# ferdean/lsa-fw

Hardware: AMD Instinct MI355X
Metric: converged eigenpairs/sec (k=20, shift-invert) (higher is better)
Workload: dtype c128

## Files before the change

### include/lsa_hip.h

```cpp
#ifndef LSA_HIP_H
#define LSA_HIP_H

#include <stdint.h>

#ifdef __cplusplus
extern "C" {
#endif

typedef enum { LSA_F64 = 0, LSA_C128 = 1 } lsa_dtype;

typedef enum {
    LSA_OK = 0,
    LSA_ERR_ARG = -1,
    LSA_ERR_HIP = -2,
    LSA_ERR_ZERO_PIVOT = -3,
    LSA_ERR_DIVERGED = -4,
    LSA_ERR_NONFINITE = -5,
    LSA_ERR_TIMEOUT = -6,
    LSA_ERR_COMM = -7,
    LSA_ERR_OOM = -8
} lsa_status;

typedef struct lsa_ctx lsa_ctx;
typedef struct lsa_mat lsa_mat;
// ... 11 lines not shown
    double max_rel_res;
    double seconds_factor;
    double seconds_solve;
    int32_t stagnated_solves;
    int32_t pc_fallback;
    int32_t backward_accepted;
    int32_t analysis_reused;
    int32_t refined_solves;
    int32_t reserved0;
} lsa_stats;

int lsa_ctx_create(int device, lsa_ctx **out);
void lsa_ctx_destroy(lsa_ctx *ctx);
const char *lsa_last_error(const lsa_ctx *ctx);
int lsa_ctx_synchronize(lsa_ctx *ctx);
int lsa_ctx_mem_info(lsa_ctx *ctx, int64_t *free_bytes, int64_t *total_bytes);
const char *lsa_ctx_arch(const lsa_ctx *ctx);

int lsa_vec_create(lsa_ctx *ctx, int64_t n, int dtype, lsa_vec **out);
void lsa_vec_destroy(lsa_vec *v);
int lsa_vec_upload(lsa_ctx *ctx, lsa_vec *v, const void *host);
int lsa_vec_download(lsa_ctx *ctx, const lsa_vec *v, void *host);

int lsa_csr_upload(lsa_ctx *ctx, int32_t n, int64_t nnz, const int32_t *rowptr, const int32_t *col,
                   const void *val, int dtype, lsa_mat **out);
void lsa_mat_destroy(lsa_mat *m);
int lsa_mat_download_values(lsa_ctx *ctx, const lsa_mat *m, void *host_val);
int lsa_csr_axpby(lsa_ctx *ctx, const lsa_mat *A, const lsa_mat *B, const double alpha[2], const double beta[2],
                  int out_dtype, lsa_mat **out);
int lsa_csr_window(lsa_ctx *ctx, const lsa_mat *M, const double *left, const double *right, lsa_mat **out);
int lsa_spmv(lsa_ctx *ctx, const lsa_mat *A, const lsa_vec *x, lsa_vec *y);
int lsa_spmv_transpose(lsa_ctx *ctx, const lsa_mat *A, int conj, const lsa_vec *x, lsa_vec *y);
int lsa_spmv_info(lsa_ctx *ctx, const lsa_mat *A, int xdtype, char *kernel, int32_t kernel_len, int64_t *bytes_moved);
int lsa_spmv_time(lsa_ctx *ctx, const lsa_mat *A, const lsa_vec *x, lsa_vec *y, int iters, double *avg_ms);

int lsa_ilu_create(lsa_ctx *ctx, const lsa_mat *C, int levels, double shift_tol, lsa_ilu **out);
void lsa_ilu_destroy(lsa_ilu *pc);
int lsa_ilu_set_algorithm(lsa_ctx *ctx, lsa_ilu *pc, int algo, int32_t block_size);
int lsa_ilu_solve(lsa_ctx *ctx, lsa_ilu *pc, int which, const lsa_vec *b, lsa_vec *x);
int lsa_ilu_solve_time(lsa_ctx *ctx, lsa_ilu *pc, int which, const lsa_vec *b, lsa_vec *x, int iters, double *avg_ms);
int lsa_ilu_info(const lsa_ilu *pc, int64_t *nnz, int32_t *levels_lower, int32_t *levels_upper, int32_t *nshift);
int lsa_ilu_download(lsa_ctx *ctx, const lsa_ilu *pc, int32_t *rowptr, int32_t *col, void *val);

typedef struct lsa_nd_sym lsa_nd_sym;
typedef struct lsa_ndlu lsa_ndlu;
int lsa_nd_analyse(int32_t n, const int32_t *rowptr, const int32_t *col, int32_t leaf_size, const int8_t *constraint, lsa_nd_sym **out);
int lsa_nd_order(int32_t n, const int32_t *rowptr, const int32_t *col, int32_t leaf_size, const int8_t *constraint, lsa_nd_sym **out);
int lsa_nd_analyse_tree(int32_t n, const int32_t *rowptr, const int32_t *col, int32_t ntree, const int32_t *first, const int32_t *size,
                        const int32_t *parent, const int32_t *owner, int32_t rank, int32_t nranks, lsa_nd_sym **out);
const char *lsa_nd_sym_error(const lsa_nd_sym *h);
void lsa_nd_sym_destroy(lsa_nd_sym *h);
int lsa_nd_sym_info(const lsa_nd_sym *h, int32_t *ntree, int32_t *nlevels, int32_t *max_front, int64_t *index_entries,
                    int64_t *factor_entries, int64_t *front_entries, double *flops);
int lsa_nd_sym_memory(const lsa_nd_sym *h, int32_t scalar_bytes, int64_t work_budget_bytes, int64_t *out, int64_t *upd_off, int64_t *work_off,
                      int32_t *chunk_of);
int lsa_nd_sym_export(const lsa_nd_sym *h, int32_t *perm, int32_t *node_start, int32_t *parent, int32_t *level, int32_t *front_size,
                      int32_t *idx);
int lsa_nd_sym_export_tables(const lsa_nd_sym *h, int32_t *cmap, int32_t *gptr, int32_t *gidx, int64_t *asm_dst, int32_t *lvl_ptr,
                             int32_t *lvl_nodes);
int lsa_nd_sym_export_dist(const lsa_nd_sym *h, int32_t *kind, int64_t *front_off, int64_t *u_off, int32_t *asm_src, int32_t *children_ptr,
                           int32_t *children_idx, int64_t *scalars);
int lsa_nd_sym_export_top(const lsa_nd_sym *h, int32_t *owner, int32_t *rows, int64_t *exch, int64_t *totals);
int lsa_ndlu_create(lsa_ctx *ctx, const lsa_mat *C, int32_t leaf_size, lsa_ndlu **out);
int lsa_ndlu_prepare(lsa_ctx *ctx, const lsa_mat *P, int dtype, int32_t leaf_size, const int8_t *constraint);
int lsa_ndlu_prepare_tree(lsa_ctx *ctx, const lsa_mat *P, int dtype, int32_t ntree, const int32_t *first, const int32_t *size,
                          const int32_t *parent);
int lsa_ndlu_create_tree(lsa_ctx *ctx, const lsa_mat *C, int32_t ntree, const int32_t *first, const int32_t *size, const int32_t *parent,
                         const int32_t *owner, lsa_ndlu **out);
int lsa_ndlu_refactor(lsa_ctx *ctx, lsa_ndlu *f, const lsa_mat *C);
void lsa_ndlu_destroy(lsa_ndlu *f);
int lsa_ndlu_solve(lsa_ctx *ctx, lsa_ndlu *f, const lsa_vec *b, lsa_vec *x);
int lsa_ndlu_solve_batch(lsa_ctx *ctx, int32_t J, lsa_ndlu *const *f, const lsa_vec *const *b, lsa_vec *const *x);
int lsa_ndlu_solve_adjoint(lsa_ctx *ctx, lsa_ndlu *f, int conj, const lsa_vec *b, lsa_vec *x);
int lsa_ndlu_solve_time(lsa_ctx *ctx, lsa_ndlu *f, const lsa_vec *b, lsa_vec *x, int iters, double *avg_ms);
int lsa_ndlu_solve_multi(lsa_ctx *ctx, lsa_ndlu *f, int trans, int32_t nrhs, const lsa_vec *B, int64_t ldb, lsa_vec *X, int64_t ldx);
int lsa_ndlu_solve_multi_time(lsa_ctx *ctx, lsa_ndlu *f, int trans, int32_t nrhs, const lsa_vec *B, int64_t ldb, lsa_vec *X, int64_t ldx,
                              int iters, double *avg_ms);
int lsa_ndlu_set_multi_transposed(lsa_ctx *ctx, lsa_ndlu *f, int on);
int lsa_ndlu_multi_info(const lsa_ndlu *f, int32_t *width, int64_t *extra_bytes, int32_t *launches_per_pass);
int lsa_ndlu_inertia(lsa_ctx *ctx, lsa_ndlu *f, int64_t *negative, int64_t *zero, int64_t *positive);
int lsa_ndlu_prepared_memory(lsa_ctx *ctx, int64_t *out);
int lsa_ndlu_info(const lsa_ndlu *f, int32_t *ntree, int32_t *nlevels, int32_t *max_front, int64_t *factor_entries,
                  int64_t *front_entries, int64_t *apply_bytes, int32_t *apply_launches, double *seconds_analyse,
                  double *seconds_numeric);
int lsa_ndlu_sweep_level(const lsa_ndlu *f, int32_t level, int32_t *nodes, int32_t *max_pivot, int32_t *fwd_rows, int32_t *bwd_rows,
                         int32_t *fwd_tiles, int32_t *bwd_tiles);

int lsa_gmres(lsa_ctx *ctx, const lsa_mat *C, lsa_ilu *pc, const lsa_vec *b, lsa_vec *x, int use_x0, double rtol,
              int restart, int maxit, int32_t *iters, double *rel_res);

typedef struct {
    int32_t ilu_levels;
    double ilu_shift;
    double ksp_rtol;
    int32_t ksp_restart;
    int32_t ksp_maxit;
    int32_t pc_type;
    double antishift[2];
} lsa_op_options;

int lsa_op_create(lsa_ctx *ctx, const lsa_mat *A, const lsa_mat *M, const double sigma[2], int mode,
                  const lsa_op_options *opts, lsa_op **out);
void lsa_op_destroy(lsa_op *op);
int lsa_op_apply(lsa_ctx *ctx, lsa_op *op, const lsa_vec *x, lsa_vec *y);
int lsa_op_stats(const lsa_op *op, lsa_stats *out);
int lsa_op_set_adjoint(lsa_ctx *ctx, lsa_op *op, int on);
int lsa_op_set_projection(lsa_ctx *ctx, lsa_op *op, const double *keep);

int lsa_krylov_create(lsa_ctx *ctx, lsa_op *op, int32_t ncv, lsa_krylov **out);
void lsa_krylov_destroy(lsa_krylov *k);
int lsa_krylov_set_row_permutation(lsa_ctx *ctx, lsa_krylov *k, const int32_t *perm);
int lsa_krylov_set_start(lsa_ctx *ctx, lsa_krylov *k, const void *host_v);
int lsa_krylov_inject(lsa_ctx *ctx, lsa_krylov *k, int32_t j, const void *host_v);
int lsa_krylov_extend(lsa_ctx *ctx, lsa_krylov *k, int32_t j0, int32_t j1, void *H, int32_t ldh, int32_t *breakdown);
int lsa_krylov_restart(lsa_ctx *ctx, lsa_krylov *k, int32_t m, int32_t knew, const void *Q, int32_t ldq);
int lsa_krylov_ritz_vectors(lsa_ctx *ctx, lsa_krylov *k, int32_t m, int32_t nvec, const void *Y, int32_t ldy,
                            int normalise, void *X);
int lsa_krylov_imag_norms(const lsa_krylov *k, int32_t nvec, double *out);
int lsa_eig_residuals(lsa_ctx *ctx, const lsa_mat *A, const lsa_mat *M, int32_t nvec, const void *lam, const void *X,
                      double *res);
int lsa_eig_biorth(lsa_ctx *ctx, const lsa_mat *M, int64_t n, int32_t nvec, const void *X, const void *Z, void *G,
                   double *norm_z, double *norm_mx);

typedef enum {
    LSA_WHICH_LARGEST_MAGNITUDE = 1,
    LSA_WHICH_LARGEST_REAL = 3,
    LSA_WHICH_SMALLEST_REAL = 4,
    LSA_WHICH_LARGEST_IMAGINARY = 5,
    LSA_WHICH_SMALLEST_IMAGINARY = 6,
    LSA_WHICH_TARGET_MAGNITUDE = 7,
    LSA_WHICH_TARGET_REAL = 8,
    LSA_WHICH_TARGET_IMAGINARY = 9
} lsa_which;
typedef struct {
    int32_t nev;
    int32_t max_restarts;
    double tol;
    int32_t which;
    int32_t transform;
    double sigma[2];
    double antishift[2];
    double target[2];
    uint64_t seed;
    double keep_fraction;
} lsa_ks_options;
typedef struct {
    int32_t nconv;
    int32_t nout;
    int32_t restarts;
    int32_t pad;
    int64_t op_applies;
    double next_unconverged;
    double seconds_expand;
    double seconds_dense;
    double seconds_restart;
} lsa_ks_result;
int lsa_krylov_shape(const lsa_krylov *k, int64_t *n, int32_t *ncv);
int64_t lsa_mat_rows(const lsa_mat *m);
int lsa_krylov_solve(lsa_ctx *ctx, lsa_krylov *k, const lsa_ks_options *opts, const void *v0, const double *mask, int32_t max_out,
                     void *theta_out, void *lambda_out, void *X_out, double *est_out, lsa_ks_result *result);
typedef struct {
    int64_t rounds;
    int64_t launches;
    int64_t periods;
    double launches_per_round;
    int64_t lockstep_steps[16];
    int64_t solo_steps[16];
// ... 137 lines not shown
```

### lsa-fw_amd/csrc/ndlu.hip

```cpp
#include "ndlu_internal.h"

namespace {

void nd_free(lsa_ndlu* f) {
    if (!f) return;
    ndlu_multi_free(f);
    for (void* p : {f->d_top, (void*)f->d_top_icmap, (void*)f->d_top_jobs, (void*)f->d_top_tiles})
        if (p) (void)hipFree(p);
    for (void* p : {(void*)f->d_lnodes_bwd, (void*)f->d_dist_nodes, (void*)f->d_child_ptr, (void*)f->d_child_idx, f->d_xstage, f->d_xg, (void*)f->d_tgoff, f->d_tg})
        if (p) (void)hipFree(p);
    for (void* p : {(void*)f->d_nodes, (void*)f->d_lnodes, (void*)f->d_gell, (void*)f->d_idx, (void*)f->d_cmap, (void*)f->d_tiles,
                    (void*)f->d_chunk_nodes, (void*)f->d_asm_dst, (void*)f->d_asm_src, (void*)f->d_ipiv, (void*)f->d_rowq, (void*)f->d_flag, (void*)f->d_xflag, (void*)f->d_maxabs,
                    f->d_lfac, f->d_ufac, f->d_work, f->d_upd, f->d_ubuf, f->d_xb, f->d_acc, f->d_tmp, f->d_ybuf, (void*)f->d_cand[0], (void*)f->d_cand[1], f->d_dinv})
        if (p) (void)hipFree(p);
    if (f->ev_panel) (void)hipEventDestroy(f->ev_panel);
    if (f->ev_pivots) (void)hipEventDestroy(f->ev_pivots);
    if (f->side) (void)hipStreamDestroy(f->side);
    delete f;
}

int nd_setup_top(lsa_ctx* ctx, lsa_ndlu* f, const std::vector<NdNodeDev>& nodes) {
    const NdSymbolic& S = f->S;
    f->top = NdTop{};
    f->top_level = -1;
// ... 14 lines not shown
        const int32_t c = S.child_idx[(size_t)c0 + ci];
        const NdNodeDev& nd = nodes[(size_t)c];
        bool on_level = false;
        for (int32_t q = S.lvl_ptr[(size_t)lr - 1]; q < S.lvl_ptr[(size_t)lr]; ++q) on_level |= S.lvl_nodes[(size_t)q] == c;
        if (!on_level || nd.nchild < 1 || nd.acc_off < 0 || nd.f <= nd.m || nd.m < 1 || S.kind[(size_t)c] == 3 || S.kind[(size_t)c] == 4) return LSA_OK;
        tp.node[ci] = NdTopNode{nd.acc_off, nd.ge_off, nd.own0, nd.m, nd.f, nd.nchild, (int32_t)s, 0};
        s += nd.m;
        replaced += (int64_t)nd.m * nd.m + 2 * (int64_t)nd.m * (nd.f - nd.m);
    }
    const NdNodeDev& nr = nodes[(size_t)R];
    tp.node[K] = NdTopNode{nr.acc_off, nr.ge_off, nr.own0, mR, mR, K, (int32_t)s, 0};
    s += mR;
    if (s > limit) return LSA_OK;
    tp.s = (int32_t)s;
    std::vector<int32_t> icmap((size_t)K * mR, -1);
    for (int32_t ci = 0; ci < K; ++ci) {
        const int32_t c = S.child_idx[(size_t)c0 + ci];
        for (int32_t p = 0; p < S.f[(size_t)c] - S.m[(size_t)c]; ++p) {
            const int32_t k = S.cmap[(size_t)S.cmap_off[(size_t)c] + p];
            if (k < 0 || k >= mR) return LSA_OK;
            icmap[(size_t)ci * mR + k] = p;
        }
    }
    std::vector<NdTopJob> jobs;
    std::vector<int32_t> tiles;
    auto add = [&](const NdTopJob& jb) {
        for (int32_t ti = 0; ti < (jb.M + 31) / 32; ++ti)
            for (int32_t tj = 0; tj < (jb.N + 31) / 32; ++tj) {
                tiles.push_back((int32_t)jobs.size());
                tiles.push_back((ti << 16) | tj);
            }
        jobs.push_back(jb);
    };
    const int64_t oR = tp.node[K].off;
    add(NdTopJob{0, 0, oR * s + oR, nr.lfac_off, mR, mR, 0, 1, 1, mR, 0, 0, 0, 0});
    for (int32_t ci = 0; ci < K; ++ci) {
        const NdNodeDev& nd = nodes[(size_t)S.child_idx[(size_t)c0 + ci]];
        const int32_t m = nd.m, b = nd.f - nd.m;
        const int64_t o = tp.node[ci].off;
        add(NdTopJob{nd.ufac_off, nr.lfac_off, o * s + oR, -1, m, mR, b, b, mR, 0, 1, 2, nd.cmap_off, 1});
        add(NdTopJob{nr.lfac_off, nd.lfac_off + (int64_t)m * m, oR * s + o, -1, mR, m, b, mR, m, 0, 0, 1, nd.cmap_off, 0});
    }
    f->top_tiles[0] = (int32_t)tiles.size() / 2;
    for (int32_t ci = 0; ci < K; ++ci)
        for (int32_t di = 0; di < K; ++di) {
            const NdNodeDev &nc = nodes[(size_t)S.child_idx[(size_t)c0 + ci]], &nd = nodes[(size_t)S.child_idx[(size_t)c0 + di]];
            add(NdTopJob{tp.node[ci].off * s + oR, nd.lfac_off + (int64_t)nd.m * nd.m, tp.node[ci].off * s + tp.node[di].off, ci == di ? nc.lfac_off : -1, nc.m,
                         nd.m, nd.f - nd.m, (int32_t)s, nd.m, nc.m, 2, 1, nd.cmap_off, 0});
        }
    f->top_tiles[1] = (int32_t)tiles.size() / 2 - f->top_tiles[0];
    LSA_CHECK(upload(ctx, icmap, &f->d_top_icmap));
    LSA_CHECK(upload(ctx, jobs, &f->d_top_jobs));
    LSA_CHECK(upload(ctx, tiles, &f->d_top_tiles));
    LSA_HIP_ALLOC(ctx, hipMalloc(&f->d_top, (size_t)(s * s) * esize(f->dtype)));
    f->top = tp;
    f->top_level = lr;
    f->top_replaced_entries = replaced;
    f->solve_launches -= 2;
    return LSA_OK;
}


struct TileBuffer {
    std::vector<int32_t> tiles;
    void begin(TileList& tl) {
        tl.off = (int64_t)tiles.size() / 2;
        tl.count = 0;
    }
    void push(TileList& tl, int32_t a, int32_t b) {
        tiles.push_back(a);
        tiles.push_back(b);
        ++tl.count;
    }
};

void nd_setup_knobs(lsa_ndlu* f) {
    const char* e = getenv("LSA_ND_TP_MIN");
    f->tp_min = e && *e ? std::max(1, atoi(e)) : 512;
    const char* sbm = getenv("LSA_ND_SB_MIN");
    f->sb_min = std::max(f->tp_min, sbm && *sbm ? std::max(1, atoi(sbm)) : 1024);
    f->ycap = kNB;
    const char* sbc = getenv("LSA_ND_SB_COLS");
    f->sb_cols = sbc && *sbc ? std::min(1024, std::max(kGT, atoi(sbc) / kGT * kGT)) : kSB;
}

bool nd_setup_ordered(const NdSymbolic& S) {
    const bool dist = S.nranks > 1;
    bool ordered = true;
    for (size_t k = 0; k < S.perm.size() && ordered; ++k) ordered = S.perm[k] == (int32_t)k || dist;
    if (dist)
        for (int32_t t = 0; t < S.nt && ordered; ++t)
            for (int32_t r = 1; r < S.m[(size_t)t]; ++r)
                if (S.idx[(size_t)S.idx_off[(size_t)t] + r] != S.idx[(size_t)S.idx_off[(size_t)t]] + r) {
                    ordered = false;
                    break;
                }
    return ordered;
}

int64_t nd_setup_budget(const NdSymbolic& S, size_t es, int64_t free_agreed) {
    size_t free_b = 0, total_b = 0;
    if (hipMemGetInfo(&free_b, &total_b) != hipSuccess) free_b = (size_t)16 << 30;
    const int64_t after = (int64_t)free_b - S.factor_entries * (int64_t)es;
    int64_t budget = std::max<int64_t>(after / 4, (int64_t)256 << 20) / (int64_t)es;
    if (S.has_dist) budget = std::max<int64_t>((free_agreed > 0 ? free_agreed : (int64_t)free_b) / 6, (int64_t)256 << 20) / (int64_t)es;
    if (const char* e = getenv("LSA_ND_WORK_MB")) budget = std::max<int64_t>(atoll(e), 1) * (1 << 20) / (int64_t)es;
    return budget;
}

std::vector<NdNodeDev> nd_setup_nodes(const NdSymbolic& S, const NdMemoryPlan& P) {
    std::vector<NdNodeDev> nodes((size_t)S.nt);
    for (int32_t t = 0; t < S.nt; ++t) {
        NdNodeDev& nd = nodes[(size_t)t];
        nd.front_off = P.work_off[(size_t)t];
        nd.lfac_off = P.lfac_off[(size_t)t];
        nd.ufac_off = P.ufac_off[(size_t)t];
        nd.upd_off = P.upd_off[(size_t)t];
        nd.u_off = S.u_off[(size_t)t];
        nd.ge_off = S.ge_off[(size_t)t];
        nd.acc_off = P.acc_off[(size_t)t];
        nd.pacc_off = P.pacc_off[(size_t)t];
        nd.idx_off = (int32_t)S.idx_off[(size_t)t];
        nd.cmap_off = S.cmap_off[(size_t)t];
        nd.piv_off = S.piv_off[(size_t)t];
        nd.own0 = S.m[(size_t)t] > 0 ? S.idx[(size_t)S.idx_off[(size_t)t]] : 0;
        nd.m = S.m[(size_t)t];
        nd.f = S.f[(size_t)t];
        nd.parent = S.parent[(size_t)t];
        nd.nchild = S.child_ptr[(size_t)t + 1] - S.child_ptr[(size_t)t];
        nd.brow0 = S.brow0[(size_t)t];
        nd.brow = S.brow[(size_t)t];
        nd.orow0 = S.orow0[(size_t)t];
        nd.orows = S.orows[(size_t)t];
        nd.flags = S.kind[(size_t)t] == 4 ? 1 : 0;
        nd.pad0 = 0;
        nd.xg_base = S.xg_base[(size_t)t];
        nd.xg_stride = S.xg_stride[(size_t)t];
        nd.inv_off = S.kind[(size_t)t] == 4
                         ? nd.front_off + (int64_t)(S.m[(size_t)t] + nd_slice_width(S.f[(size_t)t] - S.m[(size_t)t], S.nranks)) * S.f[(size_t)t]
                         : -1;
    }
    return nodes;
}

std::vector<NdChunk> nd_setup_chunks(const NdSymbolic& S, const NdMemoryPlan& P, std::vector<int32_t>& chunk_of) {
    std::vector<NdChunk> chunks;
    chunk_of.assign((size_t)S.nt, -1);
    for (size_t c = 0; c + 1 < P.chunk_begin.size(); ++c) {
        NdChunk ch;
        ch.node_begin = P.chunk_begin[c];
        ch.node_count = P.chunk_begin[c + 1] - P.chunk_begin[c];
        ch.work_entries = P.chunk_work[c];
        ch.exchange_before = P.chunk_exchange_before[c] != 0;
        for (int32_t q = 0; q < ch.node_count; ++q) {
            const int32_t t = S.lvl_nodes[(size_t)ch.node_begin + q];
            ch.max_m = std::max(ch.max_m, S.m[(size_t)t]);
            ch.max_f = std::max(ch.max_f, S.f[(size_t)t]);
            ch.sorted_m.push_back(S.m[(size_t)t]);
            chunk_of[(size_t)t] = (int32_t)c;
        }
        chunks.push_back(std::move(ch));
    }
    return chunks;
}

int nd_setup_assembly(lsa_ctx* ctx, lsa_ndlu* f, const std::vector<NdNodeDev>& nodes, const std::vector<int32_t>& chunk_of) {
// ... 603 lines not shown
}

int lsa_ndlu_solve_multi(lsa_ctx* ctx, lsa_ndlu* f, int trans, int32_t nrhs, const lsa_vec* B, int64_t ldb, lsa_vec* X, int64_t ldx) {
    LSA_CHECK(nd_multi_check(ctx, "lsa_ndlu_solve_multi", f, trans, nrhs, B, ldb, X, ldx));
    LSA_CHECK(nd_multi_run(ctx, f, trans, nrhs, B, ldb, X, ldx));
    LSA_HIP_CHECK(ctx, hipStreamSynchronize(ctx->stream));
    return LSA_OK;
}

int lsa_ndlu_solve_multi_time(lsa_ctx* ctx, lsa_ndlu* f, int trans, int32_t nrhs, const lsa_vec* B, int64_t ldb, lsa_vec* X, int64_t ldx, int iters,
                              double* avg_ms) {
    if (!avg_ms || iters < 1) return lsa_set_error(ctx, LSA_ERR_ARG, "lsa_ndlu_solve_multi_time: bad argument");
    LSA_CHECK(nd_multi_check(ctx, "lsa_ndlu_solve_multi_time", f, trans, nrhs, B, ldb, X, ldx));
    if (B->d == X->d) return lsa_set_error(ctx, LSA_ERR_ARG, "lsa_ndlu_solve_multi_time: repeated solves need B and X apart");
    LSA_CHECK(nd_multi_run(ctx, f, trans, nrhs, B, ldb, X, ldx));
    LSA_HIP_CHECK(ctx, hipEventRecord(ctx->ev0, ctx->stream));
    for (int i = 0; i < iters; ++i) LSA_CHECK(nd_multi_run(ctx, f, trans, nrhs, B, ldb, X, ldx));
    LSA_HIP_CHECK(ctx, hipEventRecord(ctx->ev1, ctx->stream));
    LSA_HIP_CHECK(ctx, hipEventSynchronize(ctx->ev1));
    float ms = 0.f;
    LSA_HIP_CHECK(ctx, hipEventElapsedTime(&ms, ctx->ev0, ctx->ev1));
    *avg_ms = (double)ms / iters;
    return LSA_OK;
}

int lsa_ndlu_set_multi_transposed(lsa_ctx* ctx, lsa_ndlu* f, int on) {
    if (!ctx || !f) return lsa_set_error(ctx, LSA_ERR_ARG, "lsa_ndlu_set_multi_transposed: null argument");
    f->multi_transposed = on != 0;
    return LSA_OK;
}

int lsa_ndlu_multi_info(const lsa_ndlu* f, int32_t* width, int64_t* extra_bytes, int32_t* launches_per_pass) {
    if (!f) return LSA_ERR_ARG;
    if (width) *width = f->multi_width;
    if (extra_bytes) *extra_bytes = f->multi_bytes;
    if (launches_per_pass) *launches_per_pass = f->solve_launches;
    return LSA_OK;
}

int lsa_ndlu_inertia(lsa_ctx* ctx, lsa_ndlu* f, int64_t* negative, int64_t* zero, int64_t* positive) {
    if (!ctx || !f || !negative || !zero || !positive) return lsa_set_error(ctx, LSA_ERR_ARG, "lsa_ndlu_inertia: null argument");
    if (f->dtype != LSA_F64) return lsa_set_error(ctx, LSA_ERR_ARG, "lsa_ndlu_inertia: needs real factors (a real symmetric matrix)");
    if (f->S.nranks != 1) return lsa_set_error(ctx, LSA_ERR_ARG, "lsa_ndlu_inertia: not available for a forest cut over ranks");
    *negative = *zero = *positive = 0;
    const NdSymbolic& S = f->S;
    std::vector<double> blk;
    LSA_HIP_CHECK(ctx, hipStreamSynchronize(ctx->stream));
    for (int32_t t = 0; t < S.nt; ++t) {
        const int32_t m = S.m[(size_t)t];
        if (m <= 0) continue;
        blk.resize((size_t)m * m);
        LSA_HIP_CHECK(ctx, hipMemcpy(blk.data(), (const double*)f->d_lfac + f->h_lfac_off[(size_t)t], (size_t)m * m * sizeof(double), hipMemcpyDeviceToHost));
        int64_t ng = 0, ze = 0, ps = 0;
        const int rc = lsa_dense_sym_inertia(m, blk.data(), m, 1e-13, &ng, &ze, &ps);
        if (rc != LSA_OK) return lsa_set_error(ctx, rc, "lsa_ndlu_inertia: the pivot block of tree node %d holds non-finite values", t);
        *negative += ng;
        *zero += ze;
        *positive += ps;
    }
    return LSA_OK;
}

int lsa_ndlu_prepared_memory(lsa_ctx* ctx, int64_t* out) {
    if (!ctx || !out) return lsa_set_error(ctx, LSA_ERR_ARG, "lsa_ndlu_prepared_memory: null argument");
    const lsa_ndlu* c = ctx->nd_cache;
    if (!c) return lsa_set_error(ctx, LSA_ERR_ARG, "lsa_ndlu_prepared_memory: the context holds no prepared analysis");
    return nd_memory_report(c->S, (int32_t)esize(c->dtype), 0, out, nullptr, nullptr, nullptr);
}

int lsa_ndlu_sweep_level(const lsa_ndlu* f, int32_t level, int32_t* nodes, int32_t* max_pivot, int32_t* fwd_rows, int32_t* bwd_rows, int32_t* fwd_tiles,
                         int32_t* bwd_tiles) {
    if (!f || level < 0 || (size_t)level >= f->levels.size()) return LSA_ERR_ARG;
    const NdLevel& L = f->levels[(size_t)level];
    if (nodes) *nodes = L.node_count;
    if (max_pivot) *max_pivot = L.max_m;
    if (fwd_rows) *fwd_rows = L.sweep_rows;
    if (bwd_rows) *bwd_rows = L.bwd_rows;
    if (fwd_tiles) *fwd_tiles = L.fwd_tiles;
    if (bwd_tiles) *bwd_tiles = L.bwd_tiles;
    return LSA_OK;
}

int lsa_ndlu_info(const lsa_ndlu* f, int32_t* ntree, int32_t* nlevels, int32_t* max_front, int64_t* factor_entries, int64_t* front_entries,
                  int64_t* apply_bytes, int32_t* apply_launches, double* seconds_analyse, double* seconds_numeric) {
    if (!f) return LSA_ERR_ARG;
    const NdSymbolic& S = f->S;
    if (ntree) *ntree = S.nt;
    if (nlevels) *nlevels = S.nlevels;
    if (max_front) {
        int32_t mf = 0;
        for (int32_t v : S.f) mf = std::max(mf, v);
        *max_front = mf;
    }
    if (factor_entries) *factor_entries = S.factor_entries;
    if (front_entries) *front_entries = f->lfac_entries + f->ufac_entries + f->work_entries + f->upd_entries;
    const int64_t swept = S.factor_entries - f->top_replaced_entries * (f->top.s > 0) + (int64_t)f->top.s * f->top.s;
    if (apply_bytes) *apply_bytes = swept * (int64_t)esize(f->dtype) + 16 * (3 * (int64_t)S.n + 2 * S.u_off[(size_t)S.nt]);
    if (apply_launches) *apply_launches = f->solve_launches;
    if (seconds_analyse) *seconds_analyse = f->seconds_analyse;
    if (seconds_numeric) *seconds_numeric = f->seconds_numeric;
    return LSA_OK;
}

}
```

### lsa-fw_amd/csrc/ndlu_factor.hip

```cpp
#include "ndlu_internal.h"

namespace {

template <typename T>
__global__ __launch_bounds__(256) void nd_maxabs2_kernel(int64_t nnz, const T* __restrict__ v, unsigned long long* __restrict__ out) {
    __shared__ double wmax[4];
    double best = 0.0;
    const int64_t stride = (int64_t)gridDim.x * blockDim.x;
    for (int64_t i = (int64_t)blockIdx.x * blockDim.x + threadIdx.x; i < nnz; i += stride) {
        const double a = s_abs2(v[i]);
        if (a == a && a > best) best = a;
        else if (a != a) best = a;
    }
    for (int o = 32; o > 0; o >>= 1) {
        const double other = __shfl_xor(best, o);
        best = (best != best) ? best : (other != other) ? other : fmax(best, other);
    }
    if ((threadIdx.x & 63) == 0) wmax[threadIdx.x >> 6] = best;
    __syncthreads();
    if (threadIdx.x == 0) {
        for (int w = 1; w < 4; ++w) best = (best != best) ? best : (wmax[w] != wmax[w]) ? wmax[w] : fmax(best, wmax[w]);
        atomicMax(out, (unsigned long long)__double_as_longlong(best));
    }
}

template <typename T>
__global__ void nd_scale_kernel(int64_t count, T* __restrict__ v, double factor) {
    const int64_t stride = (int64_t)gridDim.x * blockDim.x;
    for (int64_t i = (int64_t)blockIdx.x * blockDim.x + threadIdx.x; i < count; i += stride) v[i] = s_mul(factor, v[i]);
}

template <typename T>
__global__ void nd_assemble_kernel(int64_t count, const T* __restrict__ val, const int32_t* __restrict__ src, const int64_t* __restrict__ dst,
                                   T* __restrict__ front) {
    const int64_t stride = (int64_t)gridDim.x * blockDim.x;
    for (int64_t e = (int64_t)blockIdx.x * blockDim.x + threadIdx.x; e < count; e += stride) front[dst[e]] = val[src[e]];
}

template <typename T>
__global__ __launch_bounds__(256) void nd_extend_add_kernel(const int32_t* __restrict__ tiles, const NdNodeDev* __restrict__ nodes,
                                                            const int32_t* __restrict__ cmap, T* __restrict__ front, const T* __restrict__ upd) {
    const int32_t c = tiles[2 * blockIdx.x], i0 = tiles[2 * blockIdx.x + 1];
    const NdNodeDev nc = nodes[c];
    const NdNodeDev np = nodes[nc.parent];
    const int32_t b = nc.f - nc.m;
    const int32_t* map = cmap + nc.cmap_off;
    const int32_t i = i0 + (threadIdx.x >> 4);
    if (i >= b) return;
    const T* src = upd + nc.upd_off + (int64_t)i * b;
    int32_t pr = map[i];
    if (pr >= np.m) {
        pr -= np.brow0;
        if (pr < np.m || pr >= np.m + np.brow) return;
    }
    T* dst = front + np.front_off + (int64_t)pr * np.f;
    for (int32_t j = threadIdx.x & 15; j < b; j += 16) {
        T* d = dst + map[j];
        *d = s_add(*d, src[j]);
    }
}

template <typename T>
__global__ __launch_bounds__(256) void nd_extend_add_staged_kernel(const NdNodeDev* __restrict__ nodes, const int32_t* __restrict__ cmap, T* __restrict__ front,
                                                                   const T* __restrict__ src, int32_t c, int32_t row0, int32_t nrows) {
    const NdNodeDev nc = nodes[c];
    const NdNodeDev np = nodes[nc.parent];
    const int32_t b = nc.f - nc.m;
    const int32_t* map = cmap + nc.cmap_off;
    const int32_t k = (int32_t)blockIdx.x * 16 + (threadIdx.x >> 4);
    if (k >= nrows) return;
    int32_t pr = map[row0 + k];
    if (pr >= np.m) {
        pr -= np.brow0;
        if (pr < np.m || pr >= np.m + np.brow) return;
    }
    const T* s = src + (int64_t)k * b;
    T* dst = front + np.front_off + (int64_t)pr * np.f;
    for (int32_t j = threadIdx.x & 15; j < b; j += 16) {
        T* d = dst + map[j];
        *d = s_add(*d, s[j]);
    }
}

template <int CTRL>
__device__ __forceinline__ unsigned long long dpp_mov_key(unsigned long long v) {
    const int lo = __builtin_amdgcn_update_dpp(0, (int)(unsigned)(v & 0xFFFFFFFFull), CTRL, 0xF, 0xF, false);
    const int hi = __builtin_amdgcn_update_dpp(0, (int)(unsigned)(v >> 32), CTRL, 0xF, 0xF, false);
    return ((unsigned long long)(unsigned)hi << 32) | (unsigned)lo;
}
__device__ __forceinline__ unsigned long long wave_max_key(unsigned long long v) {
    unsigned long long o;
    o = dpp_mov_key<0xB1>(v);
    v = o > v ? o : v;
    o = dpp_mov_key<0x4E>(v);
    v = o > v ? o : v;
    o = dpp_mov_key<0x141>(v);
    v = o > v ? o : v;
    o = dpp_mov_key<0x140>(v);
    v = o > v ? o : v;
    unsigned long long best = 0ull;
#pragma unroll
    for (int row = 0; row < 4; ++row) {
        const unsigned lo = (unsigned)__builtin_amdgcn_readlane((int)(unsigned)(v & 0xFFFFFFFFull), 16 * row);
        const unsigned hi = (unsigned)__builtin_amdgcn_readlane((int)(unsigned)(v >> 32), 16 * row);
        const unsigned long long r = ((unsigned long long)hi << 32) | lo;
        best = r > best ? r : best;
    }
    return best;
}

__device__ __forceinline__ unsigned long long pivot_key(double mag2, int32_t row) {
    return ((unsigned long long)__double_as_longlong(mag2) & ~0xFFFFull) | (unsigned long long)(65535 - row);
}


template <typename T, int NT, int RPT, int W>
__global__ __launch_bounds__(NT) void nd_gj_fused_kernel(const int32_t* __restrict__ lvl_nodes, const NdNodeDev* __restrict__ nodes,
                                                         T* __restrict__ front, int32_t* __restrict__ ipiv, int32_t* __restrict__ rowq,
                                                         int32_t kb, int32_t k0, int32_t kprev, int32_t* __restrict__ flag, double tiny2) {
    __shared__ unsigned long long skey[W];
    __shared__ T prow_s[2][W];
    __shared__ int32_t prows[W];
    __shared__ T yprev[W][16];
    __shared__ int32_t pprev[W];
    const int32_t t = lvl_nodes[blockIdx.x];
    const NdNodeDev nd = nodes[t];
    const int32_t m = nd.m, ld = nd.f;
    T* a = front + nd.front_off;
    const int tid = threadIdx.x, lane = tid & 63;
    const int32_t wp = kprev >= 0 ? min(W, m - kprev) : 0;
    if (blockIdx.y > 0) {
        if (wp <= 0) return;
        const int32_t cb = ((int32_t)blockIdx.y - 1) * 16 + (tid & 15);
        const int32_t c = kb + cb;
        const bool mine = cb < kNB && c < m && !(c >= kprev && c < kprev + wp) && !(k0 >= 0 && c >= k0 && c < k0 + W);
        if (tid < W) pprev[tid] = tid < wp ? ipiv[nd.piv_off + kprev + tid] : -1;
        __syncthreads();
        for (int e = tid; e < 16 * W; e += NT) {
            const int j = e >> 4;
            yprev[j][e & 15] = (mine && j < wp) ? a[(size_t)pprev[j] * ld + c] : scalar_traits<T>::zero();
        }
        __syncthreads();
        if (!mine) return;
        T y[W];
#pragma unroll
        for (int j = 0; j < W; ++j) y[j] = yprev[j][tid & 15];
        constexpr int RL = NT / 16;
        for (int32_t i0 = tid >> 4; i0 < m; i0 += 4 * RL) {
            T cur[4], mult[4][W];
#pragma unroll
            for (int u = 0; u < 4; ++u) {
                const int32_t i = i0 + u * RL;
                const T* ai = a + (size_t)min(i, m - 1) * ld;
                cur[u] = ai[c];
#pragma unroll
                for (int j = 0; j < W; ++j) mult[u][j] = j < wp ? ai[kprev + j] : scalar_traits<T>::zero();
            }
#pragma unroll
            for (int u = 0; u < 4; ++u) {
                const int32_t i = i0 + u * RL;
                if (i >= m) break;
                bool is_piv = false;
#pragma unroll
                for (int j = 0; j < W; ++j) is_piv |= (i == pprev[j]);
                T acc = is_piv ? scalar_traits<T>::zero() : cur[u];
#pragma unroll
                for (int j = 0; j < W; ++j) fma_acc(acc, mult[u][j], y[j]);
                a[(size_t)i * ld + c] = acc;
            }
        }
        return;
    }
    if (k0 < 0) return;
    const int32_t w = min(W, m - k0);
    if (w <= 0) return;
    int32_t* piv = ipiv + nd.piv_off;
    int32_t* rq = rowq + nd.piv_off;
    if (tid < W) {
        skey[tid] = 0ull;
        pprev[tid] = tid < wp ? piv[kprev + tid] : -1;
    }
    __syncthreads();
    if (wp > 0 && tid < W * W) {
        const int j = tid / W, cc = tid % W;
        yprev[j][cc] = (j < wp && cc < w) ? a[(size_t)pprev[j] * ld + k0 + cc] : scalar_traits<T>::zero();
    }
    T r[RPT][W];
    bool used[RPT];
#pragma unroll
    for (int q = 0; q < RPT; ++q) {
        const int32_t i = tid + NT * q;
        used[q] = i >= m || rq[min(i, m - 1)] >= 0;
#pragma unroll
        for (int c = 0; c < W; ++c) r[q][c] = (i < m && c < w) ? a[(size_t)i * ld + k0 + c] : scalar_traits<T>::zero();
    }
    __syncthreads();
    if (wp > 0) {
#pragma unroll
        for (int q = 0; q < RPT; ++q) {
            const int32_t i = tid + NT * q;
            if (i >= m) continue;
            bool is_piv = false;
#pragma unroll
            for (int j = 0; j < W; ++j) is_piv |= (i == pprev[j]);
            T mult[W];
#pragma unroll
            for (int j = 0; j < W; ++j) mult[j] = j < wp ? a[(size_t)i * ld + kprev + j] : scalar_traits<T>::zero();
#pragma unroll
            for (int c = 0; c < W; ++c) {
                T acc = is_piv ? scalar_traits<T>::zero() : r[q][c];
#pragma unroll
                for (int j = 0; j < W; ++j) fma_acc(acc, mult[j], yprev[j][c]);
                r[q][c] = c < w ? acc : scalar_traits<T>::zero();
            }
        }
    }
#pragma unroll
    for (int jj = 0; jj < W; ++jj) {
        if (jj >= w) break;
        unsigned long long key = 0ull;
#pragma unroll
        for (int q = 0; q < RPT; ++q) {
            if (!used[q]) {
                const unsigned long long kq = pivot_key(s_abs2(r[q][jj]), tid + NT * q);
                key = kq > key ? kq : key;
            }
        }
        key = wave_max_key(key);
        if (lane == 0) atomicMax(&skey[jj], key);
        __syncthreads();
        key = skey[jj];
        const int32_t p = 65535 - (int32_t)(key & 0xFFFFull);
        if (tid == 0) {
            piv[k0 + jj] = p;
            prows[jj] = p;
            if (!(__longlong_as_double((long long)(key & ~0xFFFFull)) > tiny2) && atomicCAS(&flag[1], 0, t + 1) == 0) {
                flag[2] = k0 + jj;
                flag[3] = (int32_t)(key >> 32);
            }
        }
#pragma unroll
        for (int q = 0; q < RPT; ++q) {
            if (tid + NT * q == p) {
                T pv = r[q][jj];
                if (s_abs2(pv) == 0.0) s_from(pv, 1.0, 0.0);
                const T pinv = s_inv(pv);
#pragma unroll
                for (int j = 0; j < W; ++j) {
                    const T v = (j == jj) ? pinv : s_mul(pinv, r[q][j]);
                    prow_s[jj & 1][j] = v;
                    r[q][j] = v;
                }
                used[q] = true;
                rq[p] = k0 + jj;
            }
        }
        __syncthreads();
        T prow[W];
#pragma unroll
        for (int j = 0; j < W; ++j) prow[j] = prow_s[jj & 1][j];
#pragma unroll
        for (int q = 0; q < RPT; ++q) {
            const int32_t i = tid + NT * q;
            if (i >= m || i == p) continue;
            const T fm = r[q][jj];
            if (s_abs2(fm) == 0.0) continue;
            const T nfm = s_sub(scalar_traits<T>::zero(), fm);
            r[q][jj] = scalar_traits<T>::zero();
#pragma unroll
            for (int j = 0; j < W; ++j) fma_acc(r[q][j], nfm, prow[j]);
        }
    }
#pragma unroll
    for (int q = 0; q < RPT; ++q) {
        const int32_t i = tid + NT * q;
        if (i < m) {
#pragma unroll
            for (int j = 0; j < W; ++j)
                if (j < w) a[(size_t)i * ld + k0 + j] = r[q][j];
        }
    }
}

template <typename T>
__global__ __launch_bounds__(256) void nd_gj_stage_kernel(const int32_t* __restrict__ lvl_nodes, const NdNodeDev* __restrict__ nodes,
                                                          const T* __restrict__ front, const int32_t* __restrict__ ipiv, int32_t kb, int32_t kw,
                                                          int32_t ycap, int32_t c_lo, int32_t c_hi, T* __restrict__ ybuf) {
    const int32_t t = lvl_nodes[blockIdx.x];
    const NdNodeDev nd = nodes[t];
    const int32_t m = nd.m, ld = nd.f;
    const int32_t nb = min(kw, m - kb);
    const int32_t c = c_lo + (int32_t)blockIdx.y * 256 + threadIdx.x;
    if (nb <= 0 || m <= kNB || c >= min(m, c_hi)) return;
    const T* a = front + nd.front_off;
    T* yb = ybuf + (size_t)ycap * nd.piv_off;
    const int32_t* pv = ipiv + nd.piv_off + kb;
    int32_t j = 0;
    for (; j + 4 <= nb; j += 4) {
        const T v0 = a[(size_t)pv[j] * ld + c], v1 = a[(size_t)pv[j + 1] * ld + c], v2 = a[(size_t)pv[j + 2] * ld + c], v3 = a[(size_t)pv[j + 3] * ld + c];
        yb[(size_t)j * m + c] = v0;
        yb[(size_t)(j + 1) * m + c] = v1;
        yb[(size_t)(j + 2) * m + c] = v2;
        yb[(size_t)(j + 3) * m + c] = v3;
    }
    for (; j < nb; ++j) yb[(size_t)j * m + c] = a[(size_t)pv[j] * ld + c];
}

template <typename T>
__global__ __launch_bounds__(256) void nd_gj_gemm_kernel(const int32_t* __restrict__ lvl_nodes, const NdNodeDev* __restrict__ nodes,
                                                         T* __restrict__ front, const int32_t* rowq, int32_t kb,
                                                         const T* __restrict__ ybuf, int32_t only_lo, int32_t only_hi, int32_t skip_lo,
                                                         int32_t skip_hi, int32_t ztile0) {
    __shared__ T Ws[kNB][kGT + 1];
    __shared__ T Ys[kNB][kGT + 1];
    const int32_t t = lvl_nodes[blockIdx.x];
    const NdNodeDev nd = nodes[t];
    const int32_t m = nd.m, ld = nd.f;
    const int32_t nb = min(kNB, m - kb);
    const int32_t row0 = (int32_t)blockIdx.y * kGT, col0 = ((int32_t)blockIdx.z + ztile0) * kGT;
    if (nb <= 0 || row0 >= m || col0 >= m) return;
    if (col0 >= kb && col0 + kGT <= kb + nb) return;
    if (only_hi > only_lo && (col0 >= only_hi || col0 + kGT <= only_lo)) return;
    if (col0 >= skip_lo && col0 + kGT <= skip_hi) return;
    T* a = front + nd.front_off;
    const T* yb = ybuf + (size_t)kNB * nd.piv_off;
    const int32_t* rq = rowq + nd.piv_off;
    const int tid = threadIdx.x, tx = tid & 15, ty = tid >> 4;
    for (int e = tid; e < kNB * kGT; e += 256) {
        const int qa = e / kNB, ja = e - qa * kNB;
        const int32_t gr = row0 + qa;
        Ws[ja][qa] = (ja < nb && gr < m) ? a[(size_t)gr * ld + kb + ja] : scalar_traits<T>::zero();
        const int jb = e / kGT, qb = e - jb * kGT;
        const int32_t gc = col0 + qb;
        Ys[jb][qb] = (jb < nb && gc < m) ? yb[(size_t)jb * m + gc] : scalar_traits<T>::zero();
    }
    __syncthreads();
    T acc[4][4];
#pragma unroll
    for (int i = 0; i < 4; ++i)
#pragma unroll
        for (int j = 0; j < 4; ++j) acc[i][j] = scalar_traits<T>::zero();
    for (int k = 0; k < nb; ++k) {
        T av[4], bv[4];
#pragma unroll
        for (int i = 0; i < 4; ++i) av[i] = Ws[k][ty * 4 + i];
#pragma unroll
        for (int j = 0; j < 4; ++j) bv[j] = Ys[k][tx + 16 * j];
#pragma unroll
        for (int i = 0; i < 4; ++i)
#pragma unroll
            for (int j = 0; j < 4; ++j) fma_acc(acc[i][j], av[i], bv[j]);
    }
#pragma unroll
    for (int i = 0; i < 4; ++i) {
        const int32_t gr = row0 + ty * 4 + i;
        if (gr >= m) continue;
        const int32_t q = rq[gr];
        const bool is_piv = q >= kb && q < kb + nb;
#pragma unroll
        for (int j = 0; j < 4; ++j) {
            const int32_t gc = col0 + tx + 16 * j;
            if (gc >= m || (gc >= kb && gc < kb + nb)) continue;
            if ((gc >= skip_lo && gc < skip_hi) || (only_hi > only_lo && (gc < only_lo || gc >= only_hi))) continue;
            T* cptr = a + (size_t)gr * ld + gc;
            *cptr = is_piv ? acc[i][j] : s_add(*cptr, acc[i][j]);
        }
    }
}

constexpr int kTA = 8;

template <typename T>
struct tp_first {
    static constexpr int RPT = sizeof(T) == 16 ? 1 : 2;
    static constexpr int rows = 256 * RPT;
};

__host__ __device__ inline int32_t tp_sets(int32_t m, int32_t first_rows, int32_t round) {
    int32_t n = (m + first_rows - 1) / first_rows;
    for (int32_t r = 0; r < round; ++r) n = (n + kTA - 1) / kTA;
    return n;
}

template <typename T, bool FIRST, bool LAST>
__global__ __launch_bounds__(256) void nd_tp_round_kernel(const int32_t* __restrict__ lvl_nodes, const NdNodeDev* __restrict__ nodes,
                                                          const T* __restrict__ front, int32_t* __restrict__ ipiv, int32_t* __restrict__ rowq, int32_t kb,
                                                          int32_t round, const int32_t* __restrict__ cand_in, int32_t* __restrict__ cand_out,
                                                          T* __restrict__ dinv, int32_t* __restrict__ flag, double tiny2) {
// ... 193 lines not shown
    }
    T* dst = front + nd.inv_off + (size_t)ra * m;
    const bool mine = ra >= nd.orow0 && ra < nd.orow0 + nd.orows;
    T* keep = lfac + nd.lfac_off + (size_t)(mine ? ra - nd.orow0 : 0) * m;
    for (int32_t cb = threadIdx.x & 15; cb < m; cb += 16) {
        const T v = src[q[cb]];
        dst[cb] = v;
        if (mine) keep[cb] = v;
    }
}

typedef double mfma_d4 __attribute__((ext_vector_type(4)));
__device__ __forceinline__ double plane_of(double v, int) { return v; }
__device__ __forceinline__ double plane_of(cplx v, int p) { return p == 0 ? v.re : v.im; }

template <typename T>
struct MfmaTile {
    static constexpr int BK = 16, LDAS = BK + 1, LDBS = kGT + 16, NPL = (int)(sizeof(T) / sizeof(double));
    double As[NPL][kGT * LDAS];
    double Bs[NPL][BK * LDBS];
};

template <typename T, typename FA, typename FB>
__device__ __forceinline__ void mfma_tile_product(int32_t K, FA loadA, FB loadB, MfmaTile<T>& sm, mfma_d4 (&acc)[MfmaTile<T>::NPL][2][2]) {
    constexpr int BK = MfmaTile<T>::BK, LDAS = MfmaTile<T>::LDAS, LDBS = MfmaTile<T>::LDBS, NPL = MfmaTile<T>::NPL;
    const int tid = threadIdx.x, lane = tid & 63, wave = tid >> 6;
    const int wr = 32 * (wave >> 1), wc = 32 * (wave & 1), l15 = lane & 15, l4 = lane >> 4;
#pragma unroll
    for (int p = 0; p < NPL; ++p)
#pragma unroll
        for (int i = 0; i < 2; ++i)
#pragma unroll
            for (int j = 0; j < 2; ++j) acc[p][i][j] = mfma_d4{0.0, 0.0, 0.0, 0.0};
    T pa[4], pb[4];
    auto gload = [&](int32_t kk) {
#pragma unroll
        for (int s = 0; s < 4; ++s) {
            const int e = tid + 256 * s;
            pa[s] = loadA(e >> 4, kk + (e & 15));
            pb[s] = loadB(kk + (e >> 6), e & 63);
        }
    };
    gload(0);
    for (int32_t kk = 0; kk < K; kk += BK) {
#pragma unroll
        for (int s = 0; s < 4; ++s) {
            const int e = tid + 256 * s;
#pragma unroll
            for (int p = 0; p < NPL; ++p) {
                sm.As[p][(e >> 4) * LDAS + (e & 15)] = plane_of(pa[s], p);
                sm.Bs[p][(e >> 6) * LDBS + (e & 63)] = plane_of(pb[s], p);
            }
        }
        __syncthreads();
        if (kk + BK < K) gload(kk + BK);
#pragma unroll
        for (int k4 = 0; k4 < BK; k4 += 4) {
            if (kk + k4 >= K) break;
            double a[NPL][2], bb[NPL][2];
#pragma unroll
            for (int p = 0; p < NPL; ++p)
#pragma unroll
                for (int i = 0; i < 2; ++i) {
                    a[p][i] = sm.As[p][(wr + 16 * i + l15) * LDAS + k4 + l4];
                    bb[p][i] = sm.Bs[p][(k4 + l4) * LDBS + wc + 16 * i + l15];
                }
#pragma unroll
            for (int i = 0; i < 2; ++i)
#pragma unroll
                for (int j = 0; j < 2; ++j) {
                    acc[0][i][j] = __builtin_amdgcn_mfma_f64_16x16x4f64(a[0][i], bb[0][j], acc[0][i][j], 0, 0, 0);
                    if constexpr (NPL == 2) {
                        acc[0][i][j] = __builtin_amdgcn_mfma_f64_16x16x4f64(-a[NPL - 1][i], bb[NPL - 1][j], acc[0][i][j], 0, 0, 0);
                        acc[NPL - 1][i][j] = __builtin_amdgcn_mfma_f64_16x16x4f64(a[0][i], bb[NPL - 1][j], acc[NPL - 1][i][j], 0, 0, 0);
                        acc[NPL - 1][i][j] = __builtin_amdgcn_mfma_f64_16x16x4f64(a[NPL - 1][i], bb[0][j], acc[NPL - 1][i][j], 0, 0, 0);
                    }
                }
        }
        __syncthreads();
    }
}

template <typename T, int KIND>
__global__ __launch_bounds__(256) void nd_gemm_mfma_kernel(const int32_t* __restrict__ tiles, const NdNodeDev* __restrict__ nodes,
                                                           T* __restrict__ front, T* __restrict__ lfac, T* __restrict__ ufac) {
    constexpr int NPL = MfmaTile<T>::NPL;
    __shared__ MfmaTile<T> sm;
    const int32_t t = tiles[2 * blockIdx.x], packed = tiles[2 * blockIdx.x + 1];
    const int32_t tm = packed >> 16, tn = packed & 0xFFFF;
    const NdNodeDev nd = nodes[t];
    const int32_t m = nd.m, f = nd.f, b = f - m;
    T* F = front + nd.front_off;
    T* inv = nd.inv_off < 0 ? lfac + nd.lfac_off : front + nd.inv_off;
    T* invrows = lfac + nd.lfac_off;
    T* S1 = invrows + (size_t)nd.orows * m;
    T* S2 = ufac + nd.ufac_off;
    const T *A, *B;
    T* C;
    int32_t M, N, K, lda, ldb, ldc;
    if (KIND == 0) {
        A = F + (size_t)m * f, lda = f, B = inv, ldb = m, C = S1, ldc = m, M = nd.brow, N = m, K = m;
    } else if (KIND == 1) {
        A = S1, lda = m, B = F + m, ldb = f, C = F + (size_t)m * f + m, ldc = f, M = nd.brow, N = b, K = m;
    } else {
        A = invrows, lda = m, B = F + m, ldb = f, C = S2, ldc = b, M = nd.orows, N = b, K = m;
    }
    const int32_t row0 = tm * kGT, col0 = tn * kGT;
    mfma_d4 acc[NPL][2][2];
    mfma_tile_product<T>(
        K,
        [&](int r, int32_t k) {
            const int32_t gr = row0 + r;
            return (gr < M && k < K) ? A[(size_t)gr * lda + k] : scalar_traits<T>::zero();
        },
        [&](int32_t k, int c) {
            const int32_t gc = col0 + c;
            return (k < K && gc < N) ? B[(size_t)k * ldb + gc] : scalar_traits<T>::zero();
        },
        sm, acc);
    const int lane = threadIdx.x & 63, wave = threadIdx.x >> 6;
    const int wr = 32 * (wave >> 1), wc = 32 * (wave & 1), l15 = lane & 15, l4 = lane >> 4;
#pragma unroll
    for (int i = 0; i < 2; ++i)
#pragma unroll
        for (int r = 0; r < 4; ++r) {
            const int32_t gr = row0 + wr + 16 * i + l4 + 4 * r;
            if (gr >= M) continue;
#pragma unroll
            for (int j = 0; j < 2; ++j) {
                const int32_t gc = col0 + wc + 16 * j + l15;
                if (gc >= N) continue;
                T v;
                s_from(v, acc[0][i][j][r], acc[NPL - 1][i][j][r]);
                T* c = C + (size_t)gr * ldc + gc;
                if (KIND == 0) *c = s_sub(scalar_traits<T>::zero(), v);
                else if (KIND == 1) *c = s_add(*c, v);
                else *c = v;
            }
        }
}

template <typename T>
__global__ __launch_bounds__(256) void nd_gj_update_kernel(const int32_t* __restrict__ lvl_nodes, const NdNodeDev* __restrict__ nodes,
                                                           T* __restrict__ front, const int32_t* rowq, int32_t kb, int32_t kw,
                                                           const T* __restrict__ ybuf, int32_t ycap, int32_t only_lo, int32_t only_hi,
                                                           int32_t skip_lo, int32_t skip_hi, int32_t ztile0) {
    constexpr int NPL = MfmaTile<T>::NPL;
    __shared__ MfmaTile<T> sm;
    const int32_t t = lvl_nodes[blockIdx.x];
    const NdNodeDev nd = nodes[t];
    const int32_t m = nd.m, ld = nd.f;
    const int32_t nb = min(kw, m - kb);
    const int32_t row0 = (int32_t)blockIdx.y * kGT, col0 = ((int32_t)blockIdx.z + ztile0) * kGT;
    if (nb <= 0 || row0 >= m || col0 >= m) return;
    if (col0 >= kb && col0 + kGT <= kb + nb) return;
    if (only_hi > only_lo && (col0 >= only_hi || col0 + kGT <= only_lo)) return;
    if (col0 >= skip_lo && col0 + kGT <= skip_hi) return;
    T* a = front + nd.front_off;
    const T* yb = ybuf + (size_t)ycap * nd.piv_off;
    const int32_t* rq = rowq + nd.piv_off;
    mfma_d4 acc[NPL][2][2];
    mfma_tile_product<T>(
        nb,
        [&](int r, int32_t k) {
            const int32_t gr = row0 + r;
            return (gr < m && k < nb) ? a[(size_t)gr * ld + kb + k] : scalar_traits<T>::zero();
        },
        [&](int32_t k, int c) {
            const int32_t gc = col0 + c;
            return (k < nb && gc < m) ? yb[(size_t)k * m + gc] : scalar_traits<T>::zero();
        },
        sm, acc);
    const int lane = threadIdx.x & 63, wave = threadIdx.x >> 6;
    const int wr = 32 * (wave >> 1), wc = 32 * (wave & 1), l15 = lane & 15, l4 = lane >> 4;
#pragma unroll
    for (int i = 0; i < 2; ++i)
#pragma unroll
        for (int r = 0; r < 4; ++r) {
            const int32_t gr = row0 + wr + 16 * i + l4 + 4 * r;
            if (gr >= m) continue;
            const int32_t q = rq[gr];
            const bool is_piv = q >= kb && q < kb + nb;
#pragma unroll
            for (int j = 0; j < 2; ++j) {
                const int32_t gc = col0 + wc + 16 * j + l15;
                if (gc >= m || (gc >= kb && gc < kb + nb)) continue;
                if ((gc >= skip_lo && gc < skip_hi) || (only_hi > only_lo && (gc < only_lo || gc >= only_hi))) continue;
                T v;
                s_from(v, acc[0][i][j][r], acc[NPL - 1][i][j][r]);
                T* cptr = a + (size_t)gr * ld + gc;
                *cptr = is_piv ? v : s_add(*cptr, v);
            }
        }
}

template <typename T>
__global__ __launch_bounds__(256) void nd_save_update_kernel(const int32_t* __restrict__ tiles, const NdNodeDev* __restrict__ nodes,
                                                             const T* __restrict__ front, T* __restrict__ upd) {
    const int32_t t = tiles[2 * blockIdx.x], r0 = tiles[2 * blockIdx.x + 1];
    const NdNodeDev nd = nodes[t];
    const int32_t m = nd.m, f = nd.f, b = f - m;
    const int32_t r = r0 + (threadIdx.x >> 4);
    if (r >= nd.brow) return;
    const T* src = front + nd.front_off + (size_t)(m + r) * f + m;
    T* dst = upd + nd.upd_off + (size_t)r * b;
    for (int32_t c = threadIdx.x & 15; c < b; c += 16) dst[c] = src[c];
}

template <typename T>
__global__ __launch_bounds__(256) void nd_top_gemm_kernel(const int32_t* __restrict__ tiles, const NdTopJob* __restrict__ jobs,
                                                          const int32_t* __restrict__ cmap, const T* __restrict__ lfac,
                                                          const T* __restrict__ ufac, T* top, int32_t ldc) {
    __shared__ T As[16][33], Bs[16][33];
    const NdTopJob jb = jobs[tiles[2 * blockIdx.x]];
    const int32_t tile = tiles[2 * blockIdx.x + 1], i0 = (tile >> 16) * 32, j0 = (tile & 0xFFFF) * 32;
    const T* A = (jb.a_src == 0 ? lfac : jb.a_src == 1 ? ufac : (const T*)top) + jb.a_off;
    const T* B = lfac + jb.b_off;
    const int32_t* map = cmap + jb.map_off;
    const int tid = threadIdx.x, ti = tid / 16, tj = tid % 16;
    T acc[2][2] = {{scalar_traits<T>::zero(), scalar_traits<T>::zero()}, {scalar_traits<T>::zero(), scalar_traits<T>::zero()}};
    for (int32_t k0 = 0; k0 < jb.K; k0 += 16) {
#pragma unroll
        for (int h = 0; h < 2; ++h) {
            const int32_t i = i0 + ti + 16 * h, k = k0 + tj;
            As[tj][ti + 16 * h] = i < jb.M && k < jb.K ? A[(size_t)i * jb.lda + (jb.gather == 1 ? map[k] : k)] : scalar_traits<T>::zero();
            const int32_t kb = k0 + tid / 32 + 8 * h, j = j0 + tid % 32;
            Bs[tid / 32 + 8 * h][tid % 32] = kb < jb.K && j < jb.N ? B[(size_t)(jb.gather == 2 ? map[kb] : kb) * jb.ldb + j] : scalar_traits<T>::zero();
        }
        __syncthreads();
#pragma unroll
        for (int k = 0; k < 16; ++k) {
            const T a0 = As[k][ti], a1 = As[k][ti + 16], b0 = Bs[k][tj], b1 = Bs[k][tj + 16];
            fma_acc(acc[0][0], a0, b0);
            fma_acc(acc[0][1], a0, b1);
            fma_acc(acc[1][0], a1, b0);
            fma_acc(acc[1][1], a1, b1);
        }
        __syncthreads();
    }
#pragma unroll
    for (int h = 0; h < 2; ++h)
#pragma unroll
        for (int g = 0; g < 2; ++g) {
            const int32_t i = i0 + ti + 16 * h, j = j0 + tj + 16 * g;
            if (i >= jb.M || j >= jb.N) continue;
            const T d = jb.d_off >= 0 ? lfac[jb.d_off + (size_t)i * jb.ldd + j] : scalar_traits<T>::zero();
            top[jb.c_off + (size_t)i * ldc + j] = jb.negate ? s_sub(d, acc[h][g]) : s_add(d, acc[h][g]);
        }
}

template <typename T, int NT, int RPT, int W>
void launch_block(lsa_ctx* ctx, lsa_ndlu* f, const NdChunk& L, int32_t kb, double tiny2) {
    hipStream_t st = ctx->stream;
    const int32_t* lv = f->d_chunk_nodes + L.node_begin;
    T* front = (T*)f->d_work;
    auto active_at = [&](int32_t k) {
        return (int32_t)(std::lower_bound(L.sorted_m.begin(), L.sorted_m.end(), k, std::greater<int32_t>()) - L.sorted_m.begin());
    };
    const int32_t kend = std::min(kb + kNB, L.max_m);
    const bool others = std::min(kNB, L.max_m - kb) > W;
    int32_t kprev = -1, active_prev = 0;
    for (int32_t k0 = kb; k0 < kend; k0 += W) {
        const int32_t active = active_at(k0);
        if (active == 0) break;
        hipLaunchKernelGGL((nd_gj_fused_kernel<T, NT, RPT, W>), dim3(std::max(active, active_prev), others && kprev >= 0 ? 1 + kNB / 16 : 1), dim3(NT), 0, st, lv,
                           f->d_nodes, front, f->d_ipiv, f->d_rowq, kb, k0, kprev, f->d_flag, tiny2);
        kprev = k0;
        active_prev = active;
    }
    if (others && kprev >= 0)
        hipLaunchKernelGGL((nd_gj_fused_kernel<T, NT, RPT, W>), dim3(active_prev, 1 + kNB / 16), dim3(NT), 0, st, lv, f->d_nodes, front, f->d_ipiv, f->d_rowq, kb,
                           -1, kprev, f->d_flag, tiny2);
    if (L.max_m > kNB) {
        const int32_t active = active_at(kb);
        hipLaunchKernelGGL((nd_gj_stage_kernel<T>), dim3(active, (L.max_m + 255) / 256), dim3(256), 0, st, lv, f->d_nodes, (const T*)front, f->d_ipiv, kb,
                           kNB, kNB, 0, L.max_m, (T*)f->d_ybuf);
        const int32_t tiles = (L.max_m + kGT - 1) / kGT;
        hipLaunchKernelGGL((nd_gj_gemm_kernel<T>), dim3(active, tiles, tiles), dim3(256), 0, st, lv, f->d_nodes, front, f->d_rowq, kb, (const T*)f->d_ybuf, 0, 0,
                           0, 0, 0);
    }
}

template <typename T>
void launch_tournament(lsa_ndlu* f, const NdChunk& L, int32_t kb, double tiny2, hipStream_t st) {
    const int32_t* lv = f->d_chunk_nodes + L.node_begin;
    const T* front = (const T*)f->d_work;
    const int32_t active = (int32_t)(std::lower_bound(L.sorted_m.begin(), L.sorted_m.end(), kb, std::greater<int32_t>()) - L.sorted_m.begin());
    if (active == 0) return;
    int32_t sets = (L.max_m + tp_first<T>::rows - 1) / tp_first<T>::rows;
    hipLaunchKernelGGL((nd_tp_round_kernel<T, true, false>), dim3(active, sets), dim3(256), 0, st, lv, f->d_nodes, front, f->d_ipiv, f->d_rowq, kb, 0,
                       (const int32_t*)nullptr, f->d_cand[0], (T*)nullptr, f->d_flag, tiny2);
    int src = 0;
    for (int32_t round = 0;; ++round) {
        const int32_t groups = (sets + kTA - 1) / kTA;
        if (groups == 1) {
            hipLaunchKernelGGL((nd_tp_round_kernel<T, false, true>), dim3(active, 1), dim3(256), 0, st, lv, f->d_nodes, front, f->d_ipiv, f->d_rowq, kb, round,
                               (const int32_t*)f->d_cand[src], (int32_t*)nullptr, (T*)f->d_dinv, f->d_flag, tiny2);
            break;
        }
        hipLaunchKernelGGL((nd_tp_round_kernel<T, false, false>), dim3(active, groups), dim3(256), 0, st, lv, f->d_nodes, front, f->d_ipiv, f->d_rowq, kb, round,
                           (const int32_t*)f->d_cand[src], f->d_cand[src ^ 1], (T*)nullptr, f->d_flag, tiny2);
        src ^= 1;
        sets = groups;
    }
}

template <typename T>
int launch_level_tp(lsa_ctx* ctx, lsa_ndlu* f, const NdChunk& L, double tiny2) {
    hipStream_t st = ctx->stream, side = f->side;
    const int32_t* lv = f->d_chunk_nodes + L.node_begin;
    T* front = (T*)f->d_work;
    auto active_at = [&](int32_t k) {
        return (int32_t)(std::lower_bound(L.sorted_m.begin(), L.sorted_m.end(), k, std::greater<int32_t>()) - L.sorted_m.begin());
    };
    const int32_t ahead_min = getenv("LSA_ND_LOOKAHEAD_MIN") ? atoi(getenv("LSA_ND_LOOKAHEAD_MIN")) : 1024;
    const bool ahead = side != nullptr && L.max_m >= std::max(ahead_min, 2 * kNB + 1);
    const bool wide = L.max_m >= f->sb_min;
    const int32_t sbw = wide ? f->sb_cols : kNB, ycap = f->ycap;
    const int32_t tiles = (L.max_m + kGT - 1) / kGT;
    auto stage = [&](int32_t active, int32_t k0, int32_t kw, int32_t c_lo, int32_t c_hi) {
        hipLaunchKernelGGL((nd_gj_stage_kernel<T>), dim3(active, (c_hi - c_lo + 255) / 256), dim3(256), 0, st, lv, f->d_nodes, (const T*)front, f->d_ipiv, k0, kw,
                           ycap, c_lo, c_hi, (T*)f->d_ybuf);
    };
    auto update = [&](int32_t active, int32_t k0, int32_t kw, int32_t zt0, int32_t ztn, int32_t only_lo, int32_t only_hi, int32_t skip_lo, int32_t skip_hi) {
        hipLaunchKernelGGL((nd_gj_update_kernel<T>), dim3(active, tiles, ztn), dim3(256), 0, st, lv, f->d_nodes, front, f->d_rowq, k0, kw, (const T*)f->d_ybuf,
                           ycap, only_lo, only_hi, skip_lo, skip_hi, zt0);
    };
    launch_tournament<T>(f, L, 0, tiny2, st);
    for (int32_t sb0 = 0; sb0 < L.max_m; sb0 += sbw) {
        const int32_t sb1 = std::min(sb0 + sbw, L.max_m);
        if (active_at(sb0) == 0) break;
        for (int32_t kb = sb0; kb < sb1; kb += kNB) {
            const int32_t active = active_at(kb);
            if (active == 0) break;
            hipLaunchKernelGGL((nd_tp_colblock_kernel<T>), dim3(active, (L.max_m + 255) / 256), dim3(256), 0, st, lv, f->d_nodes, front, f->d_rowq, kb,
                               (const T*)f->d_dinv);
            if (sb1 - sb0 > kNB) {
                stage(active, kb, kNB, sb0, sb1);
                update(active, kb, kNB, sb0 / kGT, (sb1 + kGT - 1) / kGT - sb0 / kGT, sb0, sb1, 0, 0);
                if (kb + kNB < sb1 && active_at(kb + kNB) > 0) launch_tournament<T>(f, L, kb + kNB, tiny2, st);
            }
        }
        const int32_t active = active_at(sb0), next = sb1;
        const bool has_next = next < L.max_m && active_at(next) > 0;
        if (L.max_m > sb1 - sb0) {
            stage(active, sb0, sb1 - sb0, 0, L.max_m);
            if (has_next && ahead) {
                update(active, sb0, sb1 - sb0, next / kGT, 1, next, next + kNB, 0, 0);
                LSA_HIP_CHECK(ctx, hipEventRecord(f->ev_panel, st));
                LSA_HIP_CHECK(ctx, hipStreamWaitEvent(side, f->ev_panel, 0));
                launch_tournament<T>(f, L, next, tiny2, side);
                LSA_HIP_CHECK(ctx, hipEventRecord(f->ev_pivots, side));
                update(active, sb0, sb1 - sb0, 0, tiles, 0, 0, next, next + kNB);
                LSA_HIP_CHECK(ctx, hipStreamWaitEvent(st, f->ev_pivots, 0));
                continue;
            }
            update(active, sb0, sb1 - sb0, 0, tiles, 0, 0, 0, 0);
        }
        if (has_next) launch_tournament<T>(f, L, next, tiny2, st);
    }
    return LSA_OK;
}

template <typename T>
int nd_numeric(lsa_ctx* ctx, lsa_ndlu* f, const lsa_mat* C) {
    const NdSymbolic& S = f->S;
    hipStream_t st = ctx->stream;
    T* front = (T*)f->d_work;
    T* lfac = (T*)f->d_lfac;
    T* ufac = (T*)f->d_ufac;
    T* upd = (T*)f->d_upd;
    int rc0 = LSA_OK;
    double max2 = 0.0;
    {
        auto head = [&]() -> int {
            LSA_HIP_CHECK(ctx, hipMemsetAsync(f->d_rowq, 0xFF, (size_t)std::max<int32_t>(S.n, 1) * sizeof(int32_t), st));
            LSA_HIP_CHECK(ctx, hipMemsetAsync(f->d_flag, 0, 4 * sizeof(int32_t), st));
            LSA_HIP_CHECK(ctx, hipMemsetAsync(f->d_maxabs, 0, sizeof(unsigned long long), st));
            if (S.nnz > 0) {
                const int blocks = (int)std::min<int64_t>((S.nnz + 255) / 256, (int64_t)ctx->num_cu * 2);
                hipLaunchKernelGGL((nd_maxabs2_kernel<T>), dim3(blocks), dim3(256), 0, st, S.nnz, (const T*)C->val, f->d_maxabs);
            }
            unsigned long long mbits = 0;
            LSA_HIP_CHECK(ctx, hipMemcpyAsync(&mbits, f->d_maxabs, sizeof mbits, hipMemcpyDeviceToHost, st));
            LSA_HIP_CHECK(ctx, hipStreamSynchronize(st));
            memcpy(&max2, &mbits, sizeof max2);
            if (!std::isfinite(max2)) return lsa_set_error(ctx, LSA_ERR_NONFINITE, "lsa_ndlu: the matrix holds non-finite values");
            return LSA_OK;
        };
        rc0 = S.nranks > 1 ? k_agree_status(ctx, head()) : head();
        if (rc0 != LSA_OK) return rc0;
    }
    const double tiny2 = 1e-30 * max2;
    const int32_t* tl = f->d_tiles;
    bool exchanged = false;
    for (size_t ci = 0; ci < f->chunks.size(); ++ci) {
        const NdChunk& L = f->chunks[ci];
        if (L.exchange_before && f->xupd_slot > 0) {
            LSA_CHECK(k_allgather_inplace(ctx, f->d_upd, (size_t)f->xupd_slot * sizeof(T)));
            exchanged = true;
        }
        LSA_HIP_CHECK(ctx, hipMemsetAsync(f->d_work, 0, (size_t)L.work_entries * sizeof(T), st));
        if (L.asm_count > 0) {
            const int blocks = (int)std::min<int64_t>((L.asm_count + 255) / 256, (int64_t)ctx->num_cu * 16);
            hipLaunchKernelGGL((nd_assemble_kernel<T>), dim3(blocks), dim3(256), 0, st, L.asm_count, (const T*)C->val, f->d_asm_src + L.asm_begin,
                               f->d_asm_dst + L.asm_begin, front);
        }
        for (const TileList& e : L.ext)
            if (e.count > 0)
                hipLaunchKernelGGL((nd_extend_add_kernel<T>), dim3(e.count), dim3(256), 0, st, tl + 2 * e.off, f->d_nodes, f->d_cmap, front, (const T*)upd);
        for (const auto& step : L.xsteps) {
            T* stage = (T*)f->d_xstage;
            int64_t stride = 0;
            for (int r = 0; r < S.nranks; ++r) {
                const NdChunk::XPiece& pc = step[(size_t)r];
                if (pc.nrows > 0) stride = std::max(stride, (int64_t)pc.nrows * (S.f[(size_t)pc.child] - S.m[(size_t)pc.child]));
            }
            if (stride == 0) continue;
            const NdChunk::XPiece& mine = step[(size_t)S.rank];
            if (mine.nrows > 0) {
                const int32_t bc = S.f[(size_t)mine.child] - S.m[(size_t)mine.child];
                const int64_t src_off = f->chunk_node_upd_off(mine.child) + (int64_t)(mine.row0 - S.brow0[(size_t)mine.child]) * bc;
                LSA_HIP_CHECK(ctx, hipMemcpyAsync(stage + (size_t)S.rank * (size_t)stride, upd + src_off, (size_t)mine.nrows * (size_t)bc * sizeof(T),
                                                  hipMemcpyDeviceToDevice, st));
            }
            LSA_CHECK(k_allgather_inplace(ctx, stage, (size_t)stride * sizeof(T)));
            for (int r = 0; r < S.nranks; ++r) {
                const NdChunk::XPiece& pc = step[(size_t)r];
                if (pc.nrows <= 0) continue;
                hipLaunchKernelGGL((nd_extend_add_staged_kernel<T>), dim3((pc.nrows + 15) / 16), dim3(256), 0, st, f->d_nodes, f->d_cmap, front,
                                   (const T*)(stage + (size_t)r * (size_t)stride), pc.child, pc.row0, pc.nrows);
            }
        }
        if (L.max_m >= f->tp_min) LSA_CHECK(launch_level_tp<T>(ctx, f, L, tiny2));
        for (int32_t kb = 0; kb < L.max_m && L.max_m < f->tp_min; kb += kNB) {
            if (L.max_m <= 64) launch_block<T, 64, 1, 8>(ctx, f, L, kb, tiny2);
            else if (L.max_m <= 128) launch_block<T, 128, 1, 8>(ctx, f, L, kb, tiny2);
            else if (L.max_m <= 256) launch_block<T, 256, 1, 8>(ctx, f, L, kb, tiny2);
            else if (L.max_m <= 512) launch_block<T, 512, 1, 8>(ctx, f, L, kb, tiny2);
            else if (L.max_m <= 1024) launch_block<T, 1024, 1, 8>(ctx, f, L, kb, tiny2);
            else if (L.max_m <= 2048) launch_block<T, 1024, 2, 8>(ctx, f, L, kb, tiny2);
            else if (L.max_m <= 4096) launch_block<T, 1024, 4, 4>(ctx, f, L, kb, tiny2);
            else if (L.max_m <= 8192) launch_block<T, 1024, 8, 2>(ctx, f, L, kb, tiny2);
            else launch_block<T, 1024, 16, 1>(ctx, f, L, kb, tiny2);
        }
        if (L.unperm.count > 0)
            hipLaunchKernelGGL((nd_unperm_kernel<T>), dim3(L.unperm.count), dim3(256), 0, st, tl + 2 * L.unperm.off, f->d_nodes, front, f->d_ipiv,
                               f->d_rowq, lfac);
        auto product = [&](auto kind) {
            constexpr int KIND = decltype(kind)::value;
            if (L.gemm[KIND].count == 0) return;
            hipLaunchKernelGGL((nd_gemm_mfma_kernel<T, KIND>), dim3(L.gemm[KIND].count), dim3(256), 0, st, tl + 2 * L.gemm[KIND].off, f->d_nodes, front, lfac, ufac);
        };
        product(std::integral_constant<int, 0>{});
        product(std::integral_constant<int, 1>{});
        product(std::integral_constant<int, 2>{});
        if (L.save.count > 0)
            hipLaunchKernelGGL((nd_save_update_kernel<T>), dim3(L.save.count), dim3(256), 0, st, tl + 2 * L.save.off, f->d_nodes, (const T*)front, upd);
    }
    if (f->top.s > 0)
        for (int q = 0, t0 = 0; q < 2; t0 += f->top_tiles[q++])
            if (f->top_tiles[q] > 0)
                hipLaunchKernelGGL((nd_top_gemm_kernel<T>), dim3(f->top_tiles[q]), dim3(256), 0, st, f->d_top_tiles + 2 * t0, f->d_top_jobs, f->d_cmap,
                                   (const T*)lfac, (const T*)ufac, (T*)f->d_top, f->top.s);
    if (!exchanged && S.nranks > 1 && f->xupd_slot > 0)
        LSA_CHECK(k_allgather_inplace(ctx, f->d_upd, (size_t)f->xupd_slot * sizeof(T)));
    int32_t hflag[4] = {0, 0, 0, 0};
    if (S.nranks > 1) {
        LSA_HIP_CHECK(ctx, hipMemcpyAsync(f->d_xflag + 4 * S.rank, f->d_flag, 4 * sizeof(int32_t), hipMemcpyDeviceToDevice, st));
        LSA_CHECK(k_allgather_inplace(ctx, f->d_xflag, 4 * sizeof(int32_t)));
        std::vector<int32_t> all((size_t)4 * S.nranks, 0);
        LSA_HIP_CHECK(ctx, hipMemcpyAsync(all.data(), f->d_xflag, all.size() * sizeof(int32_t), hipMemcpyDeviceToHost, st));
        LSA_HIP_CHECK(ctx, hipStreamSynchronize(st));
        for (int r = 0; r < S.nranks; ++r)
            if (all[(size_t)4 * r + 1] != 0) {
                memcpy(hflag, &all[(size_t)4 * r], sizeof hflag);
                if (r != S.rank) hflag[1] = -(r + 1);
                break;
            }
    } else {
        LSA_HIP_CHECK(ctx, hipMemcpyAsync(hflag, f->d_flag, sizeof hflag, hipMemcpyDeviceToHost, st));
        LSA_HIP_CHECK(ctx, hipStreamSynchronize(st));
    }
    LSA_HIP_CHECK(ctx, hipGetLastError());
    if (hflag[1] < 0)
        return lsa_set_error(ctx, LSA_ERR_ZERO_PIVOT, "lsa_ndlu: a pivot block on rank %d is singular to 1e-15 * max|C| (column %d of its node)", -hflag[1] - 1,
                             hflag[2]);
    if (hflag[1] != 0) {
        const int32_t t = hflag[1] - 1;
        const unsigned long long hi = (unsigned long long)(uint32_t)hflag[3] << 32;
        double mag2;
        memcpy(&mag2, &hi, sizeof mag2);
        return lsa_set_error(ctx, LSA_ERR_ZERO_PIVOT,
                             "lsa_ndlu: the pivot block of tree node %d (%d unknowns, front %d, level %d) is singular at its column %d: largest "
                             "candidate pivot %.3e against max|C| = %.3e (threshold 1e-15 max|C|); the matrix is singular, or needs pivoting "
                             "across fronts",
                             t, S.m[(size_t)t], S.f[(size_t)t], S.level[(size_t)t], hflag[2], std::sqrt(mag2), std::sqrt(max2));
    }
    if (const char* pe = getenv("LSA_ND_TEST_PERTURB")) {
        const double eps = atof(pe);
        if (eps != 0.0 && f->ufac_entries > 0) {
            const int blocks = (int)std::min<int64_t>((f->ufac_entries + 255) / 256, (int64_t)ctx->num_cu * 16);
            hipLaunchKernelGGL((nd_scale_kernel<T>), dim3(blocks), dim3(256), 0, st, f->ufac_entries, ufac, 1.0 + eps);
            LSA_HIP_CHECK(ctx, hipStreamSynchronize(st));
        }
    }
    return LSA_OK;
}

}

int ndlu_numeric(lsa_ctx* ctx, lsa_ndlu* f, const lsa_mat* C) {
    return f->dtype == LSA_C128 ? nd_numeric<cplx>(ctx, f, C) : nd_numeric<double>(ctx, f, C);
}
```

### lsa-fw_amd/csrc/ndlu_internal.h

```cpp
#pragma once
#include <algorithm>
#include <chrono>
#include <cmath>
#include <cstdlib>
#include <functional>
#include <new>
#include <string>

#include "lsa_internal.h"
#include "nd_internal.h"

int k_allgather_inplace(lsa_ctx* ctx, void* vec, size_t bytes_per_rank);

constexpr int kRT = 32;
constexpr int kSweepWide = 512;
constexpr int kCH = 1024;
constexpr int kGT = 64;
constexpr int kNB = 32;
constexpr int kSB = 128;
constexpr int kTRmin = 256;
constexpr int kNdBatchMax = 16;
static_assert(kNdBatchMax == kKrylovGroupMax, "a lockstep round hands all its problems to one batched sweep");
constexpr int kMCH = 256;
constexpr int kNdMultiMax = 8;
// ... 40 lines not shown
    int64_t off = 0;
    int32_t count = 0;
};

struct NdChunk {
    int32_t node_begin = 0, node_count = 0, max_m = 0, max_f = 0;
    std::vector<int32_t> sorted_m;
    int64_t work_entries = 0;
    int64_t asm_begin = 0, asm_count = 0;
    TileList unperm, gemm[3], save;
    std::vector<TileList> ext;
    bool exchange_before = false;
    struct XPiece {
        int32_t child = -1, row0 = 0, nrows = 0;
    };
    std::vector<std::vector<XPiece>> xsteps;
};

struct NdLevel {
    int32_t node_begin = 0, node_count = 0, max_m = 0, max_f = 0;
    int32_t fwd_tiles = 0, bwd_tiles = 0;
    int32_t sweep_rows = 32;
    int32_t bwd_rows = 32;
    int32_t dist_begin = 0, dist_count = 0, dist_children = 0, dist_rows = 0;
    int64_t ux_base = 0, ux_slot = 0, xg_base = 0, xg_slot = 0;
};

constexpr int kTopChildren = 8;
struct NdTopNode {
    int64_t acc_off, ge_off;
    int32_t own0, m, f, nchild;
    int32_t off, pad0;
};
struct NdTop {
    int32_t s, nchild;
    NdTopNode node[kTopChildren + 1];
};

struct NdTopJob {
    int64_t a_off, b_off, c_off, d_off;
    int32_t M, N, K, lda, ldb, ldd;
    int32_t a_src, gather;
    int32_t map_off, negate;
};
static_assert(sizeof(NdTopJob) == 72, "assembly job layout");

struct lsa_ndlu {
    lsa_ctx* ctx = nullptr;
    NdSymbolic S;
    int dtype = LSA_C128;
    bool ordered = false;
    std::vector<NdChunk> chunks;
    std::vector<NdLevel> levels;
    NdNodeDev* d_nodes = nullptr;
    NdSweepNode *d_lnodes = nullptr, *d_lnodes_bwd = nullptr;
    int32_t *d_dist_nodes = nullptr, *d_child_ptr = nullptr, *d_child_idx = nullptr;
    void *d_xstage = nullptr, *d_xg = nullptr;
    int64_t* d_tgoff = nullptr;
    void* d_tg = nullptr;
    std::vector<int64_t> tg_slot;
    int64_t tg_slot_max = 0;
    int64_t xstage_slot = 0;
    std::vector<int64_t> h_upd_off, h_lfac_off;
    int64_t chunk_node_upd_off(int32_t t) const { return h_upd_off[(size_t)t]; }
    int32_t* d_gell = nullptr;
    int32_t *d_idx = nullptr, *d_cmap = nullptr, *d_tiles = nullptr, *d_chunk_nodes = nullptr;
    int64_t* d_asm_dst = nullptr;
    int32_t* d_asm_src = nullptr;
    int64_t asm_count = 0;
    int32_t *d_ipiv = nullptr, *d_rowq = nullptr, *d_flag = nullptr, *d_xflag = nullptr;
    unsigned long long* d_maxabs = nullptr;
    void *d_lfac = nullptr, *d_ufac = nullptr;
    void *d_work = nullptr, *d_upd = nullptr;
    void *d_ubuf = nullptr, *d_xb = nullptr, *d_acc = nullptr;
    void *d_tmp = nullptr, *d_ybuf = nullptr;
    int64_t lfac_entries = 0, ufac_entries = 0, work_entries = 0, upd_entries = 0, acc_entries = 0;
    int64_t xupd_slot = 0;
    int32_t *d_cand[2] = {nullptr, nullptr};
    void* d_dinv = nullptr;
    int32_t tp_min = 1 << 30;
    int32_t sb_min = 1 << 30;
    int32_t sb_cols = 128;
    int32_t ycap = 32;
    hipStream_t side = nullptr;
    hipEvent_t ev_panel = nullptr, ev_pivots = nullptr;
    double seconds_analyse = 0.0, seconds_numeric = 0.0;
    int32_t solve_launches = 0;
    NdTop top = {};
    int32_t top_level = -1;
    void* d_top = nullptr;
    int32_t* d_top_icmap = nullptr;
    NdTopJob* d_top_jobs = nullptr;
    int32_t* d_top_tiles = nullptr;
    int32_t top_tiles[2] = {0, 0};
    int64_t top_replaced_entries = 0;
    int acc_vbytes = 0;
    struct MultiColumn {
        void *ubuf = nullptr, *xb = nullptr, *acc = nullptr, *tmp = nullptr;
        int acc_vbytes = 0;
    };
    std::vector<MultiColumn> multi;
    bool multi_full = false;
    int64_t multi_bytes = 0;
    int32_t multi_width = 0;
    bool multi_transposed = false;
};

template <typename U>
int upload(lsa_ctx* ctx, const std::vector<U>& h, U** d) {
    const size_t bytes = std::max<size_t>(h.size(), 1) * sizeof(U);
    LSA_HIP_ALLOC(ctx, hipMalloc((void**)d, bytes));
    if (!h.empty()) LSA_HIP_CHECK(ctx, hipMemcpy(*d, h.data(), h.size() * sizeof(U), hipMemcpyHostToDevice));
    return LSA_OK;
}

int ndlu_numeric(lsa_ctx* ctx, lsa_ndlu* f, const lsa_mat* C);
bool nd_batch_compatible(const lsa_ndlu* f, const lsa_ndlu* g);
int ndlu_solve_batch_dev(lsa_ctx* ctx, int32_t J, lsa_ndlu* const* f, int vdtype, const void** b, void* const* x);
int ndlu_solve_multi_dev(lsa_ctx* ctx, lsa_ndlu* f, int vdtype, int32_t nrhs, const void* B, int64_t ldb, void* X, int64_t ldx);
void ndlu_multi_free(lsa_ndlu* f);
```

### lsa-fw_amd/csrc/solver.hip

```cpp
#include <algorithm>
#include <chrono>
#include <cmath>
#include <complex>

#include "lsa_internal.h"

int ilu_check_abort(lsa_ctx* ctx, lsa_ilu* pc);
bool nd_batch_compatible(const lsa_ndlu* f, const lsa_ndlu* g);
int ndlu_solve_batch_dev(lsa_ctx* ctx, int32_t J, lsa_ndlu* const* f, int vdtype, const void** b, void* const* x);
int k_allgather_inplace(lsa_ctx* ctx, void* vec, size_t bytes_per_rank);

namespace {

using zc = std::complex<double>;
inline size_t esize(int dtype) { return dtype == LSA_C128 ? 16 : 8; }
inline double now_s() {
    return std::chrono::duration<double>(std::chrono::steady_clock::now().time_since_epoch()).count();
}

struct KrylovSwitches {
    bool fused;
    bool four_passes;
    bool tail;
    bool delayed;
// ... 541 lines not shown
    op->owned = op->owned_diag = nullptr;
    op->pc = nullptr;
    op->opts = *opts;
    op->sigma[0] = sigma[0];
    op->sigma[1] = sigma[1];
    op->gw_ready = false;
    op->t = nullptr;
    memset(&op->st, 0, sizeof op->st);
    const bool zshift = sigma[0] == 0.0 && sigma[1] == 0.0;
    const bool cdt = sigma[1] != 0.0 || A->dtype == LSA_C128 || (M && M->dtype == LSA_C128);
    int rc = LSA_OK;
    lsa_mat* C = nullptr;
    if (!(mode == 1 && zshift)) {
        rc = build_shifted(ctx, A, M, sigma, cdt, &C);
        if (rc != LSA_OK) {
            delete op;
            return rc;
        }
        op->owned = C;
    }
    const lsa_mat* fac_src = nullptr;
    if (mode == 0 || mode == 2) {
        op->Kfac = C;
        op->Kmul = M;
        op->M_whole = M;
        bool shard_rows = false;
        if (tree) {
            const char* e = getenv("LSA_DIST_SPMV");
            shard_rows = (e && *e) ? (e[0] == 's') : (C->nnz > 60 * (int64_t)C->n);
        }
        if (tree && shard_rows) {
            op->view_fac = mat_row_view(C, tree->row0, tree->row1);
            op->Kfac = op->view_fac;
            if (M) {
                op->view_mul = mat_row_view(M, tree->row0, tree->row1);
                op->Kmul = op->view_mul;
            }
        }
        if (mode == 2) {
            const double mnu[2] = {-opts->antishift[0], -opts->antishift[1]};
            const bool cmul = cdt || opts->antishift[1] != 0.0;
            rc = build_shifted(ctx, A, M, mnu, cmul, &op->owned_mul);
            if (rc != LSA_OK) {
                lsa_op_destroy(op);
                return rc;
            }
            if (tree && shard_rows) {
                if (op->view_mul) lsa_mat_destroy(op->view_mul);
                op->view_mul = mat_row_view(op->owned_mul, tree->row0, tree->row1);
                op->Kmul = op->view_mul;
            } else op->Kmul = op->owned_mul;
        }
        if (sharded) {
            rc = build_shifted(ctx, Ad, Md, sigma, cdt, &op->owned_diag);
            if (rc != LSA_OK) {
                lsa_op_destroy(op);
                return rc;
            }
            fac_src = op->owned_diag;
        } else fac_src = C;
    } else {
        op->Kmul = C ? C : A;
        op->Kfac = M;
        fac_src = sharded ? Md : M;
    }
    bool lu_fell_back = false;
    if (opts->pc_type == 3) {
        lsa_op_destroy(op);
        return lsa_set_error(ctx, LSA_ERR_ARG, "lsa_op_create: pc_type 3 (the banded block LU of round 1) left the product library; it lives on as a "
                                               "cross-check library for the tests (tests/xcheck).  Use pc_type 2, the nested-dissection LU");
    }
    if (op->Kfac && fac_src && opts->pc_type == 2) {
        if (tree) {
            rc = lsa_ndlu_create_tree(ctx, fac_src, tree->nt, tree->first, tree->size, tree->parent, tree->owner, &op->nd);
            op->nd_dist = rc == LSA_OK;
            if (rc == LSA_ERR_OOM) {
                lsa_op_destroy(op);
                return rc;
            }
        } else
            rc = lsa_ndlu_create(ctx, fac_src, 0, &op->nd);
        if (rc == LSA_OK && op->nd) {
            double sa = 1.0;
            (void)lsa_ndlu_info(op->nd, nullptr, nullptr, nullptr, nullptr, nullptr, nullptr, nullptr, &sa, nullptr);
            op->st.analysis_reused = sa == 0.0 ? 1 : 0;
        }
        if (rc == LSA_ERR_OOM) {
            fprintf(stderr, "[lsa_hip] exact LU does not fit the device memory (%s): falling back to ILU(%d) + GMRES\n", ctx->err.c_str(),
                    opts->ilu_levels);
            lu_fell_back = true;
            op->st.pc_fallback = 1;
        } else if (rc != LSA_OK) {
            lsa_op_destroy(op);
            return rc;
        }
    }
    if (op->Kfac && fac_src && (opts->pc_type == 1 || lu_fell_back)) {
        rc = lsa_ilu_create(ctx, fac_src, opts->ilu_levels, opts->ilu_shift, &op->pc);
        if (rc != LSA_OK) {
            lsa_op_destroy(op);
            return rc;
        }
    }
    const size_t tb = (size_t)std::max<int64_t>(op->n, 1) * 16;
    if (hipMalloc(&op->t, tb) != hipSuccess || hipMemsetAsync(op->t, 0, tb, ctx->stream) != hipSuccess) {
        lsa_op_destroy(op);
        return lsa_set_error(ctx, LSA_ERR_HIP, "lsa_op_create: out of device memory");
    }
    if (op->Kfac && op->nd && fac_src && fac_src->nnz > 0) {
        double* nr = (double*)op->t;
        double v2 = 0.0;
        if (k_nrm2(ctx, fac_src->dtype, fac_src->nnz, fac_src->val, nr) == LSA_OK &&
            hipMemcpyAsync(&v2, nr, sizeof v2, hipMemcpyDeviceToHost, ctx->stream) == hipSuccess && hipStreamSynchronize(ctx->stream) == hipSuccess &&
            std::isfinite(v2))
            op->normF = std::sqrt(v2);
        (void)hipMemsetAsync(op->t, 0, sizeof(double), ctx->stream);
    }
    op->st.seconds_factor = now_s() - t0;
    *out = op;
    return LSA_OK;
}

int lsa_op_create(lsa_ctx* ctx, const lsa_mat* A, const lsa_mat* M, const double sigma[2], int mode, const lsa_op_options* opts,
                  lsa_op** out) {
    return op_build(ctx, A, M, nullptr, nullptr, sigma, mode, opts, out);
}

int lsa_op_create_sharded(lsa_ctx* ctx, const lsa_mat* A_rows, const lsa_mat* M_rows, const lsa_mat* A_diag, const lsa_mat* M_diag,
                          const double sigma[2], int mode, const lsa_op_options* opts, lsa_op** out) {
    if (!A_diag) return lsa_set_error(ctx, LSA_ERR_ARG, "lsa_op_create_sharded: the diagonal block of A is required");
    return op_build(ctx, A_rows, M_rows, A_diag, M_diag, sigma, mode, opts, out);
}

int lsa_op_create_dist(lsa_ctx* ctx, const lsa_mat* A, const lsa_mat* M, int32_t row0, int32_t row1, int32_t ntree, const int32_t* first,
                       const int32_t* size, const int32_t* parent, const int32_t* owner, const double sigma[2], int mode, const lsa_op_options* opts,
                       lsa_op** out) {
    if (!first || !size || !parent || !owner || ntree < 1) return lsa_set_error(ctx, LSA_ERR_ARG, "lsa_op_create_dist: the forest is required");
    const TreeArg tree{ntree, first, size, parent, owner, row0, row1};
    return op_build(ctx, A, M, nullptr, nullptr, sigma, mode, opts, out, &tree);
}

void lsa_op_destroy(lsa_op* op) {
    if (!op) return;
    if (op->ctx && op->ctx->stream) (void)hipStreamSynchronize(op->ctx->stream);
    if (op->pc) lsa_ilu_destroy(op->pc);
    if (op->nd) lsa_ndlu_destroy(op->nd);
    if (op->view_fac) lsa_mat_destroy(op->view_fac);
    if (op->view_mul) lsa_mat_destroy(op->view_mul);
    if (op->owned) lsa_mat_destroy(op->owned);
    if (op->owned_mul) lsa_mat_destroy(op->owned_mul);
    if (op->owned_diag) lsa_mat_destroy(op->owned_diag);
    if (op->gw_ready) op->gw.release();
    if (op->t) (void)hipFree(op->t);
    if (op->keep) (void)hipFree(op->keep);
    delete op;
}

static int op_apply_dev(lsa_ctx* ctx, lsa_op* op, const void* x, void* y) {
    const int dtype = LSA_C128;
    ++op->st.op_applies;
    const void* rhs = x;
    if (op->Kmul) {
        void* dst = op->Kfac ? op->t : y;
        LSA_CHECK(spmv_global(ctx, op->Kmul, dtype, x, dst, op->adjoint));
        ++op->st.spmv_calls;
        rhs = dst;
    }
// ... 632 lines not shown
    LSA_HIP_ALLOC(ctx, hipMalloc((void**)&gb->tail_parts, cells * 2 * (size_t)gb->nparts * sizeof(double)));
    LSA_HIP_CHECK(ctx, hipMemsetAsync(gb->tail_parts, 0, cells * 2 * (size_t)gb->nparts * sizeof(double), ctx->stream));
    return LSA_OK;
}

void krylov_group_free(KrylovGroupBuf* gb) {
    for (void* p : {gb->Hdev, (void*)gb->checks, (void*)gb->tail_parts})
        if (p) (void)hipFree(p);
    memset(gb, 0, sizeof *gb);
}

int krylov_group_check(lsa_ctx* ctx, int32_t J, lsa_krylov* const* ks) {
    for (int32_t z = 0; z < J; ++z) {
        if (!ks[z] || !ks[z]->op) return lsa_set_error(ctx, LSA_ERR_ARG, "lsa_krylov_solve_batch: null workspace (problem %d)", z);
        if (ks[z]->ctx != ctx) return lsa_set_error(ctx, LSA_ERR_ARG, "lsa_krylov_solve_batch: the workspace of problem %d lives in another context", z);
        if (ks[z]->n != ks[0]->n || ks[z]->ncv != ks[0]->ncv || ks[z]->batch != ks[0]->batch)
            return lsa_set_error(ctx, LSA_ERR_ARG, "lsa_krylov_solve_batch: problem %d has another shape (n = %lld, ncv = %d) than problem 0 (n = %lld, ncv = %d)", z,
                                 (long long)ks[z]->n, ks[z]->ncv, (long long)ks[0]->n, ks[0]->ncv);
        for (int32_t y = 0; y < z; ++y)
            if (ks[y] == ks[z] || ks[y]->op == ks[z]->op)
                return lsa_set_error(ctx, LSA_ERR_ARG, "lsa_krylov_solve_batch: problems %d and %d share a workspace or an operator", y, z);
    }
    return LSA_OK;
}

int krylov_extend_batch(lsa_ctx* ctx, KrylovGroupBuf* gb, lsa_krylov* const* ks, const uint8_t* active, const int32_t* j0, int32_t j1, void* const* Hs,
                        int32_t ldh, int32_t* breakdown, int32_t* status, std::string* errs, lsa_ks_batch_info* info) {
    const int32_t J = gb->J, slots = gb->slots;
    const double t0 = now_s();
    auto fail = [&](int32_t z, int rc) {
        status[z] = rc;
        lsa_name_problem(ctx, z);
        errs[z] = ctx->err;
    };
    struct Member {
        ExtendCursor c;
        HessView H;
        bool lock;
        int32_t nb;
    } mem[kKrylovGroupMax];
    int32_t nactive = 0;
    int32_t ncv = 0;
    for (int32_t z = 0; z < J; ++z) {
        mem[z] = Member{ExtendCursor{0, false}, HessView{nullptr, 0, 0, 0}, false, 0};
        if (!active[z]) continue;
        ++nactive;
        ncv = ks[z]->ncv;
        breakdown[z] = -1;
        status[z] = LSA_OK;
        mem[z] = Member{ExtendCursor{j0[z], false}, HessView{(cplx*)Hs[z], ldh, j0[z], ks[z]->ncv}, true, 0};
        ks[z]->t_for = -1;
        ks[z]->drop_preapply();
    }
    const size_t colb = krylov_slot_bytes(ncv);
    const size_t cells = (size_t)J * (size_t)slots;
    while (true) {
        int32_t lead = -1, rounds = 0;
        for (int32_t z = 0; z < J; ++z) {
            Member& m = mem[z];
            m.nb = 0;
            if (!active[z] || !m.lock || status[z] != LSA_OK || breakdown[z] >= 0 || m.c.j >= j1) continue;
            lsa_krylov* k = ks[z];
            const StepPlan plan = step_plan(ctx, k);
            bool in = plan.pipelined && plan.orth == Orth::dcgs2 && plan.tail;
            if (in && lead >= 0)
                in = nd_batch_compatible(ks[lead]->op->nd, k->op->nd) && ks[lead]->op->Kmul->dtype == k->op->Kmul->dtype;
            if (!in) {
                m.lock = false;
                continue;
            }
            int rc = pipelined_prepare(ctx, k, plan);
            if (rc == LSA_OK) rc = k->ow.ensure_fused(ctx, k->n);
            if (rc != LSA_OK) {
                fail(z, rc);
                continue;
            }
            if (lead < 0) lead = z;
            m.nb = std::min<int32_t>(slots, j1 - m.c.j);
            rounds = std::max(rounds, m.nb);
        }
        if (lead < 0) break;
        int rc = lsa_ensure_scratch(ctx, 0, cells * (colb + 2 * sizeof(double)));
        int32_t sweep_launches = 0;
        (void)lsa_ndlu_info(ks[lead]->op->nd, nullptr, nullptr, nullptr, nullptr, nullptr, nullptr, &sweep_launches, nullptr, nullptr);
        for (int32_t s = 0; s < rounds && rc == LSA_OK; ++s) {
            int32_t R = 0, jr[kKrylovGroupMax], fr[kKrylovGroupMax];
            lsa_ndlu* nd[kKrylovGroupMax];
            const lsa_mat *Mr[kKrylovGroupMax], *Cr[kKrylovGroupMax];
            const void *rhs[kKrylovGroupMax], *yr[kKrylovGroupMax];
            void *xr[kKrylovGroupMax], *Vr[kKrylovGroupMax], *slot[kKrylovGroupMax], *work[kKrylovGroupMax], *tr[kKrylovGroupMax];
            double* parts[kKrylovGroupMax];
            int32_t products = 0;
            for (int32_t z = 0; z < J && rc == LSA_OK; ++z) {
                if (s >= mem[z].nb) continue;
                lsa_krylov* k = ks[z];
                lsa_op* op = k->op;
                const int32_t j = mem[z].c.j + s;
                const size_t cell = (size_t)s * (size_t)J + (size_t)z;
                if (k->t_for != j) {
                    rc = spmv_global(ctx, op->Kmul, LSA_C128, (char*)k->V + (size_t)j * (size_t)k->n * 16, op->t, false);
                    ++products;
                }
                k->t_for = -1;
                jr[R] = j;
                fr[R] = (s == 0 && !mem[z].c.pending) ? 1 : 0;
                nd[R] = op->nd;
                Mr[R] = op->Kmul;
                Cr[R] = op->Kfac;
                rhs[R] = op->t;
                xr[R] = k->w;
                yr[R] = k->w;
                Vr[R] = k->V;
                slot[R] = (char*)gb->Hdev + cell * colb;
                work[R] = k->ow.fused;
                tr[R] = op->t;
                parts[R] = gb->tail_parts + cell * 2 * (size_t)gb->nparts;
                ++R;
            }
            if (rc == LSA_OK) rc = ndlu_solve_batch_dev(ctx, R, nd, LSA_C128, rhs, xr);
            if (rc == LSA_OK) rc = k_dcgs2_step_batch(ctx, R, ks[lead]->n, jr, Vr, ks[lead]->n, yr, fr, slot, ncv, work);
            if (rc == LSA_OK) rc = k_dcgs2_tail_batch(ctx, R, ks[lead]->n, jr, Vr, ks[lead]->n, yr, work, Mr, Cr, tr, parts, slot, ncv);
            for (int32_t z = 0; z < J; ++z)
                if (s < mem[z].nb) ks[z]->t_for = mem[z].c.j + s + 1;
            if (info) {
                ++info->rounds;
                info->launches += sweep_launches + 3 + products;
            }
        }
        if (rc == LSA_OK) rc = k_cgs2_tail_checks(ctx, rounds * J, gb->nparts, gb->tail_parts, gb->checks);
        char* host = (char*)ctx->pinned;
        if (rc == LSA_OK && (hipMemcpyAsync(host, gb->Hdev, (size_t)rounds * J * colb, hipMemcpyDeviceToHost, ctx->stream) != hipSuccess ||
                             hipMemcpyAsync(host + cells * colb, gb->checks, (size_t)rounds * J * 2 * sizeof(double), hipMemcpyDeviceToHost, ctx->stream) != hipSuccess))
            rc = lsa_set_error(ctx, LSA_ERR_HIP, "lsa_krylov_solve_batch: read-back of a period failed");
        if (hipStreamSynchronize(ctx->stream) != hipSuccess && rc == LSA_OK) rc = lsa_set_error(ctx, LSA_ERR_HIP, "lsa_krylov_solve_batch: a lockstep period failed on the device");
        if (info) ++info->periods;
        if (rc != LSA_OK) {
            const std::string text = ctx->err;
            for (int32_t z = 0; z < J; ++z)
                if (mem[z].nb > 0) {
                    ctx->err = text;
                    fail(z, rc);
                }
            break;
        }
        const double* chk = (const double*)(host + cells * colb);
        for (int32_t z = 0; z < J; ++z) {
            Member& m = mem[z];
            if (m.nb == 0) continue;
            int32_t accepted = 0;
            const int arc = accept_steps(ctx, ks[z], m.H, true, host + (size_t)z * colb, (size_t)J * colb, chk + 2 * (size_t)z, 2 * (size_t)J, m.nb, &m.c,
                                         &breakdown[z], &accepted);
            if (breakdown[z] >= 0) accepted = breakdown[z] + 1 - m.c.j;
            if (arc != LSA_OK) fail(z, arc);
            else if (info) info->lockstep_steps[z] += accepted;
        }
    }
    for (int32_t z = 0; z < J; ++z) {
        if (!active[z] || status[z] != LSA_OK || breakdown[z] >= 0) continue;
        const int32_t jb = mem[z].c.j;
        const int xrc = extend_rest(ctx, ks[z], mem[z].H, &mem[z].c, j1, &breakdown[z]);
        if (xrc != LSA_OK) fail(z, xrc);
        else if (info) info->solo_steps[z] += (breakdown[z] >= 0 ? breakdown[z] + 1 : j1) - jb;
    }
    const double share = (now_s() - t0) / std::max(nactive, 1);
    for (int32_t z = 0; z < J; ++z)
        if (active[z]) ks[z]->op->st.seconds_solve += share;
    return LSA_OK;
// ... 132 lines not shown
```

### lsa-fw_amd/lsa_hip/__init__.py

```python

from __future__ import annotations

import ctypes
import os
from pathlib import Path

import numpy as np

LSA_F64, LSA_C128 = 0, 1

_STATUS_NAMES = {
    0: "LSA_OK",
    -1: "LSA_ERR_ARG",
    -2: "LSA_ERR_HIP",
    -3: "LSA_ERR_ZERO_PIVOT",
    -4: "LSA_ERR_DIVERGED",
    -5: "LSA_ERR_NONFINITE",
    -6: "LSA_ERR_TIMEOUT",
    -7: "LSA_ERR_COMM",
    -8: "LSA_ERR_OOM",
}

globals().update({name: code for code, name in _STATUS_NAMES.items()})

# ... 102 lines not shown
        ("seconds_factor", ctypes.c_double),
        ("seconds_solve", ctypes.c_double),
        ("seconds_product", ctypes.c_double),
        ("seconds_gram", ctypes.c_double),
        ("seconds_dense", ctypes.c_double),
        ("solver", lsa_stats),
    ]


class lsa_stochastic_stats(ctypes.Structure):
    _fields_ = [
        ("nodes", ctypes.c_int32),
        ("kind", ctypes.c_int32),
        ("bytes", ctypes.c_int64),
        ("seconds_factor", ctypes.c_double),
        ("seconds_solve", ctypes.c_double),
        ("seconds_product", ctypes.c_double),
        ("seconds_dense", ctypes.c_double),
        ("solver", lsa_stats),
    ]


_P = ctypes.c_void_p
_I32, _I64, _DBL = ctypes.c_int32, ctypes.c_int64, ctypes.c_double
_PP = ctypes.POINTER(ctypes.c_void_p)

SIGNATURES = {
    "lsa_ctx_create": (ctypes.c_int, [ctypes.c_int, _PP]),
    "lsa_ctx_destroy": (None, [_P]),
    "lsa_last_error": (ctypes.c_char_p, [_P]),
    "lsa_ctx_synchronize": (ctypes.c_int, [_P]),
    "lsa_ctx_mem_info": (ctypes.c_int, [_P, ctypes.POINTER(_I64), ctypes.POINTER(_I64)]),
    "lsa_ctx_arch": (ctypes.c_char_p, [_P]),
    "lsa_vec_create": (ctypes.c_int, [_P, _I64, ctypes.c_int, _PP]),
    "lsa_vec_destroy": (None, [_P]),
    "lsa_vec_upload": (ctypes.c_int, [_P, _P, _P]),
    "lsa_vec_download": (ctypes.c_int, [_P, _P, _P]),
    "lsa_csr_upload": (ctypes.c_int, [_P, _I32, _I64, _P, _P, _P, ctypes.c_int, _PP]),
    "lsa_mat_destroy": (None, [_P]),
    "lsa_mat_download_values": (ctypes.c_int, [_P, _P, _P]),
    "lsa_csr_axpby": (ctypes.c_int, [_P, _P, _P, _DBL * 2, _DBL * 2, ctypes.c_int, _PP]),
    "lsa_csr_window": (ctypes.c_int, [_P, _P, _P, _P, _PP]),
    "lsa_spmv": (ctypes.c_int, [_P, _P, _P, _P]),
    "lsa_spmv_transpose": (ctypes.c_int, [_P, _P, ctypes.c_int, _P, _P]),
    "lsa_spmv_info": (ctypes.c_int, [_P, _P, ctypes.c_int, ctypes.c_char_p, _I32, ctypes.POINTER(_I64)]),
    "lsa_spmv_time": (ctypes.c_int, [_P, _P, _P, _P, ctypes.c_int, ctypes.POINTER(_DBL)]),
    "lsa_ilu_create": (ctypes.c_int, [_P, _P, ctypes.c_int, _DBL, _PP]),
    "lsa_ilu_destroy": (None, [_P]),
    "lsa_ilu_set_algorithm": (ctypes.c_int, [_P, _P, ctypes.c_int, _I32]),
    "lsa_ilu_solve": (ctypes.c_int, [_P, _P, ctypes.c_int, _P, _P]),
    "lsa_ilu_solve_time": (ctypes.c_int, [_P, _P, ctypes.c_int, _P, _P, ctypes.c_int, ctypes.POINTER(_DBL)]),
    "lsa_ilu_info": (ctypes.c_int, [_P, ctypes.POINTER(_I64), ctypes.POINTER(_I32), ctypes.POINTER(_I32), ctypes.POINTER(_I32)]),
    "lsa_ilu_download": (ctypes.c_int, [_P, _P, _P, _P, _P]),
    "lsa_nd_analyse": (ctypes.c_int, [_I32, _P, _P, _I32, _P, _PP]),
    "lsa_nd_order": (ctypes.c_int, [_I32, _P, _P, _I32, _P, _PP]),
    "lsa_nd_analyse_tree": (ctypes.c_int, [_I32, _P, _P, _I32, _P, _P, _P, _P, _I32, _I32, _PP]),
    "lsa_nd_sym_export_dist": (ctypes.c_int, [_P, _P, _P, _P, _P, _P, _P, _P]),
    "lsa_nd_sym_export_top": (ctypes.c_int, [_P, _P, _P, _P, _P]),
    "lsa_ndlu_inertia": (ctypes.c_int, [_P, _P, ctypes.POINTER(_I64), ctypes.POINTER(_I64), ctypes.POINTER(_I64)]),
    "lsa_dense_sym_inertia": (ctypes.c_int, [_I32, _P, _I32, _DBL, ctypes.POINTER(_I64), ctypes.POINTER(_I64), ctypes.POINTER(_I64)]),
    "lsa_nd_sym_error": (ctypes.c_char_p, [_P]),
    "lsa_nd_sym_destroy": (None, [_P]),
    "lsa_nd_sym_info": (ctypes.c_int, [_P, ctypes.POINTER(_I32), ctypes.POINTER(_I32), ctypes.POINTER(_I32), ctypes.POINTER(_I64),
                                       ctypes.POINTER(_I64), ctypes.POINTER(_I64), ctypes.POINTER(_DBL)]),
    "lsa_nd_sym_export": (ctypes.c_int, [_P, _P, _P, _P, _P, _P, _P]),
    "lsa_nd_sym_memory": (ctypes.c_int, [_P, _I32, _I64, _P, _P, _P, _P]),
    "lsa_nd_sym_export_tables": (ctypes.c_int, [_P, _P, _P, _P, _P, _P, _P]),
    "lsa_ndlu_create": (ctypes.c_int, [_P, _P, _I32, _PP]),
    "lsa_ndlu_prepare": (ctypes.c_int, [_P, _P, ctypes.c_int, _I32, _P]),
    "lsa_ndlu_prepare_tree": (ctypes.c_int, [_P, _P, ctypes.c_int, _I32, _P, _P, _P]),
    "lsa_ndlu_create_tree": (ctypes.c_int, [_P, _P, _I32, _P, _P, _P, _P, _PP]),
    "lsa_ndlu_refactor": (ctypes.c_int, [_P, _P, _P]),
    "lsa_ndlu_destroy": (None, [_P]),
    "lsa_ndlu_solve": (ctypes.c_int, [_P, _P, _P, _P]),
    "lsa_ndlu_solve_batch": (ctypes.c_int, [_P, _I32, _PP, _PP, _PP]),
    "lsa_ndlu_prepared_memory": (ctypes.c_int, [_P, _P]),
    "lsa_ndlu_solve_adjoint": (ctypes.c_int, [_P, _P, ctypes.c_int, _P, _P]),
    "lsa_ndlu_solve_time": (ctypes.c_int, [_P, _P, _P, _P, ctypes.c_int, ctypes.POINTER(_DBL)]),
    "lsa_ndlu_solve_multi": (ctypes.c_int, [_P, _P, ctypes.c_int, _I32, _P, _I64, _P, _I64]),
    "lsa_ndlu_solve_multi_time": (ctypes.c_int, [_P, _P, ctypes.c_int, _I32, _P, _I64, _P, _I64, ctypes.c_int, ctypes.POINTER(_DBL)]),
    "lsa_ndlu_set_multi_transposed": (ctypes.c_int, [_P, _P, ctypes.c_int]),
    "lsa_ndlu_multi_info": (ctypes.c_int, [_P, ctypes.POINTER(_I32), ctypes.POINTER(_I64), ctypes.POINTER(_I32)]),
    "lsa_ndlu_info": (ctypes.c_int, [_P, ctypes.POINTER(_I32), ctypes.POINTER(_I32), ctypes.POINTER(_I32), ctypes.POINTER(_I64),
                                     ctypes.POINTER(_I64), ctypes.POINTER(_I64), ctypes.POINTER(_I32), ctypes.POINTER(_DBL), ctypes.POINTER(_DBL)]),
    "lsa_ndlu_sweep_level": (ctypes.c_int, [_P, _I32] + [ctypes.POINTER(_I32)] * 6),
    "lsa_gmres": (ctypes.c_int, [_P, _P, _P, _P, _P, ctypes.c_int, _DBL, ctypes.c_int, ctypes.c_int, ctypes.POINTER(_I32), ctypes.POINTER(_DBL)]),
    "lsa_op_create": (ctypes.c_int, [_P, _P, _P, _DBL * 2, ctypes.c_int, ctypes.POINTER(lsa_op_options), _PP]),
    "lsa_op_create_sharded": (ctypes.c_int, [_P, _P, _P, _P, _P, _DBL * 2, ctypes.c_int, ctypes.POINTER(lsa_op_options), _PP]),
    "lsa_op_create_dist": (ctypes.c_int, [_P, _P, _P, _I32, _I32, _I32, _P, _P, _P, _P, _DBL * 2, ctypes.c_int, ctypes.POINTER(lsa_op_options), _PP]),
    "lsa_op_destroy": (None, [_P]),
    "lsa_op_apply": (ctypes.c_int, [_P, _P, _P, _P]),
    "lsa_op_stats": (ctypes.c_int, [_P, ctypes.POINTER(lsa_stats)]),
    "lsa_op_set_adjoint": (ctypes.c_int, [_P, _P, ctypes.c_int]),
    "lsa_op_set_projection": (ctypes.c_int, [_P, _P, _P]),
    "lsa_krylov_create": (ctypes.c_int, [_P, _P, _I32, _PP]),
    "lsa_krylov_destroy": (None, [_P]),
    "lsa_krylov_set_row_permutation": (ctypes.c_int, [_P, _P, _P]),
    "lsa_krylov_set_start": (ctypes.c_int, [_P, _P, _P]),
    "lsa_krylov_inject": (ctypes.c_int, [_P, _P, _I32, _P]),
    "lsa_krylov_extend": (ctypes.c_int, [_P, _P, _I32, _I32, _P, _I32, ctypes.POINTER(_I32)]),
    "lsa_krylov_restart": (ctypes.c_int, [_P, _P, _I32, _I32, _P, _I32]),
    "lsa_krylov_ritz_vectors": (ctypes.c_int, [_P, _P, _I32, _I32, _P, _I32, ctypes.c_int, _P]),
    "lsa_krylov_imag_norms": (ctypes.c_int, [_P, _I32, _P]),
    "lsa_krylov_shape": (ctypes.c_int, [_P, ctypes.POINTER(_I64), ctypes.POINTER(_I32)]),
    "lsa_mat_rows": (_I64, [_P]),
    "lsa_krylov_solve": (ctypes.c_int, [_P, _P, _P, _P, _P, _I32, _P, _P, _P, _P, _P]),
    "lsa_krylov_solve_batch": (ctypes.c_int, [_P, _I32, _PP, _PP, _PP, _I32, _PP, _PP, _PP, _PP, _P, _P, _P]),
    "lsa_eigs_sinvert": (ctypes.c_int, [_P, _P, _P, _DBL * 2, _I32, _I32, _DBL, _I32, ctypes.POINTER(lsa_op_options), _P, _P, _I32, _P, _P, _P, _P, _P]),
    "lsa_dense_schur": (ctypes.c_int, [_I32, _P, _I32, _P, _I32]),
    "lsa_dense_schur_reorder": (ctypes.c_int, [_I32, _P, _I32, _P, _I32, _P, ctypes.POINTER(_I32)]),
    "lsa_dense_tri_eigenvectors": (ctypes.c_int, [_I32, _P, _I32, _P, _I32]),
    "lsa_eig_residuals": (ctypes.c_int, [_P, _P, _P, _I32, _P, _P, _P]),
    "lsa_eig_biorth": (ctypes.c_int, [_P, _P, _I64, _I32, _P, _P, _P, _P, _P]),
    "lsa_lanczos_create": (ctypes.c_int, [_P, _P, _I32, _PP]),
    "lsa_lanczos_destroy": (None, [_P]),
    "lsa_lanczos_set_row_permutation": (ctypes.c_int, [_P, _P, _P]),
    "lsa_lanczos_set_start": (ctypes.c_int, [_P, _P, _P]),
    "lsa_lanczos_extend": (ctypes.c_int, [_P, _P, _I32, _I32, _P, _I32, ctypes.POINTER(_I32)]),
    "lsa_lanczos_basis": (ctypes.c_int, [_P, _P, _I32, _P]),
    "lsa_lanczos_solve": (ctypes.c_int, [_P, _P, ctypes.POINTER(lsa_ks_options), _P, _I32, _P, _P, _P, _P, ctypes.POINTER(lsa_ks_result)]),
    "lsa_dense_syev": (ctypes.c_int, [_I32, _P, _I32, _P]),
    "lsa_resolvent_create": (ctypes.c_int, [_P, _P, _I32, _PP]),
    "lsa_resolvent_destroy": (None, [_P]),
    "lsa_resolvent_set_row_permutation": (ctypes.c_int, [_P, _P, _P]),
    "lsa_resolvent_set_block_forcings": (ctypes.c_int, [_P, _P, ctypes.c_int]),
    "lsa_resolvent_set_weights": (ctypes.c_int, [_P, _P, _P, _P]),
    "lsa_resolvent_set_start": (ctypes.c_int, [_P, _P, _P]),
    "lsa_resolvent_extend": (ctypes.c_int, [_P, _P, _I32, _I32, _P, _I32, ctypes.POINTER(_I32)]),
    "lsa_resolvent_basis": (ctypes.c_int, [_P, _P, _I32, _P]),
    "lsa_resolvent_solve": (ctypes.c_int, [_P, _P, ctypes.POINTER(lsa_ks_options), _P, _I32, _P, _P, _P, _P, _P, ctypes.POINTER(lsa_ks_result), _P]),
    "lsa_growth_create": (ctypes.c_int, [_P, _P, _I32, _I32, _P, _PP]),
    "lsa_growth_destroy": (None, [_P]),
    "lsa_growth_set_row_permutation": (ctypes.c_int, [_P, _P, _P]),
    "lsa_growth_set_steps": (ctypes.c_int, [_P, _P, _I32]),
    "lsa_growth_set_scheme": (ctypes.c_int, [_P, _P, _I32]),
    "lsa_growth_set_response_weight": (ctypes.c_int, [_P, _P, _P]),
    "lsa_growth_response_energy": (ctypes.c_int, [_P, _P, _I32, _P]),
    "lsa_growth_set_start": (ctypes.c_int, [_P, _P, _P]),
    "lsa_growth_extend": (ctypes.c_int, [_P, _P, _I32, _I32, _P, _I32, ctypes.POINTER(_I32)]),
    "lsa_growth_basis": (ctypes.c_int, [_P, _P, _I32, _P]),
    "lsa_growth_solve": (ctypes.c_int, [_P, _P, ctypes.POINTER(lsa_ks_options), _P, _I32, _P, _P, _P, _P, _P, _P, ctypes.POINTER(lsa_ks_result), _P]),
    "lsa_spmm": (ctypes.c_int, [_P, _P, _I32, _P, _I64, _P, _I64]),
    "lsa_block_gram": (ctypes.c_int, [_P, _I64, _I32, _P, _I64, _I32, _P, _I64, _P]),
    "lsa_contour_create": (ctypes.c_int, [_P, _P, _P, _I32, _DBL * 2, _DBL * 2, _I32, ctypes.c_int, _DBL, _PP]),
    "lsa_contour_destroy": (None, [_P]),
    "lsa_contour_set_row_permutation": (ctypes.c_int, [_P, _P, _P]),
    "lsa_contour_solve": (ctypes.c_int, [_P, _P, _DBL, _I32, _P, _I32, _P, _P, _P, ctypes.POINTER(lsa_contour_result)]),
    "lsa_contour_info": (ctypes.c_int, [_P, ctypes.POINTER(lsa_contour_stats)]),
    "lsa_shifted_spmm": (ctypes.c_int, [_P, _P, _P, _I32, _P, _P, _P]),
    "lsa_stochastic_create": (ctypes.c_int, [_P, _P, _P, _I32, _P, _P, _I32, _DBL, _PP]),
    "lsa_stochastic_destroy": (None, [_P]),
    "lsa_stochastic_set_row_permutation": (ctypes.c_int, [_P, _P, _P]),
    "lsa_stochastic_set_weights": (ctypes.c_int, [_P, _P, _P, _P]),
    "lsa_stochastic_set_kind": (ctypes.c_int, [_P, _P, _I32]),
    "lsa_stochastic_set_batch_forward": (ctypes.c_int, [_P, _P, ctypes.c_int]),
    "lsa_stochastic_set_refinement": (ctypes.c_int, [_P, _P, ctypes.c_int]),
    "lsa_stochastic_apply": (ctypes.c_int, [_P, _P, _P, _P, _P]),
    "lsa_stochastic_solve": (ctypes.c_int, [_P, _P, ctypes.POINTER(lsa_ks_options), _P, _I32, _P, _P, _P, ctypes.POINTER(lsa_ks_result), _P]),
    "lsa_stochastic_info": (ctypes.c_int, [_P, ctypes.POINTER(lsa_stochastic_stats)]),
    "lsa_mm_open": (ctypes.c_int, [ctypes.c_char_p, _PP, ctypes.POINTER(_I32), ctypes.POINTER(_I32), ctypes.POINTER(_I64), ctypes.POINTER(ctypes.c_int)]),
    "lsa_mm_read_csr": (ctypes.c_int, [_P, _P, _P, _P]),
    "lsa_mm_error": (ctypes.c_char_p, [_P]),
    "lsa_mm_close": (None, [_P]),
    "lsa_comm_unique_id": (ctypes.c_int, [_P]),
    "lsa_comm_init": (ctypes.c_int, [_P, ctypes.c_int, ctypes.c_int, _P]),
    "lsa_comm_init_host": (ctypes.c_int, [_P, ctypes.c_int, ctypes.c_int, _P, _P]),
    "lsa_comm_stats": (ctypes.c_int, [_P, ctypes.POINTER(_I64), ctypes.POINTER(_I64)]),
# ... 379 lines not shown
        upd = np.zeros(self.ntree, np.int64) if detail else None
        work = np.zeros(self.ntree, np.int64) if detail else None
        chunk = np.full(self.ntree, -1, np.int32) if detail else None
        rc = self._lib.lsa_nd_sym_memory(self.handle, int(scalar_bytes), int(work_budget_bytes), _ptr(out), None if upd is None else _ptr(upd),
                                         None if work is None else _ptr(work), None if chunk is None else _ptr(chunk))
        if rc != 0:
            raise ValueError("lsa_nd_sym_memory: bad argument")
        rec = {"factors": int(out[0]), "working_arena": int(out[1]), "update_arena": int(out[2]), "exchange_region": int(out[3]), "sweep_buffers": int(out[4]),
               "chunks": int(out[5]), "largest_front": int(out[6]), "index_tables": int(out[7])}
        rec["total"] = rec["factors"] + rec["working_arena"] + rec["update_arena"] + rec["sweep_buffers"] + rec["index_tables"]
        if detail:
            rec.update({"upd_off": upd, "work_off": work, "chunk_of": chunk})
        return rec

    def export_tables(self) -> dict:
        ex = self.export()
        m = np.diff(ex["node_start"])
        b = ex["front_size"] - m
        scal = np.zeros(6, np.int64)
        self._lib.lsa_nd_sym_export_dist(self.handle, None, None, None, None, None, None, _ptr(scal))
        nlist = int(np.count_nonzero(np.ones(self.ntree)))
        out = {"cmap": np.empty(int(b.sum()), np.int32), "gptr": np.empty(int((ex["front_size"] + 1).sum()), np.int32),
               "gidx": np.empty(int(b.sum()), np.int32), "asm_dst": np.empty(int(scal[3]), np.int64), "lvl_ptr": np.empty(self.nlevels + 1, np.int32),
               "lvl_nodes": np.full(nlist, -1, np.int32), "kind": np.empty(self.ntree, np.int32), "front_off": np.empty(self.ntree + 1, np.int64),
               "u_off": np.empty(self.ntree + 1, np.int64), "asm_src": np.empty(int(scal[3]), np.int32), "child_ptr": np.empty(self.ntree + 1, np.int32)}
        self._lib.lsa_nd_sym_export_tables(self.handle, *[_ptr(out[k]) for k in ("cmap", "gptr", "gidx", "asm_dst", "lvl_ptr", "lvl_nodes")])
        out["lvl_nodes"] = out["lvl_nodes"][: int(out["lvl_ptr"][-1])]
        self._lib.lsa_nd_sym_export_dist(self.handle, _ptr(out["kind"]), _ptr(out["front_off"]), _ptr(out["u_off"]), _ptr(out["asm_src"]),
                                         _ptr(out["child_ptr"]), None, None)
        out["child_idx"] = np.empty(int(out["child_ptr"][-1]), np.int32)
        self._lib.lsa_nd_sym_export_dist(self.handle, None, None, None, None, None, _ptr(out["child_idx"]), None)
        out["owner"] = np.zeros(self.ntree, np.int32)
        rows, exch, totals = np.zeros(4 * self.ntree, np.int32), np.zeros(4 * self.ntree, np.int64), np.zeros(2, np.int64)
        self._lib.lsa_nd_sym_export_top(self.handle, _ptr(out["owner"]), _ptr(rows), _ptr(exch), _ptr(totals))
        rows, exch = rows.reshape(-1, 4), exch.reshape(-1, 4)
        out.update({"brow0": rows[:, 0].copy(), "brow": rows[:, 1].copy(), "orow0": rows[:, 2].copy(), "orows": rows[:, 3].copy(),
                    "ux_base": exch[:, 0].copy(), "ux_stride": exch[:, 1].copy(), "xg_base": exch[:, 2].copy(), "xg_stride": exch[:, 3].copy(),
                    "u_entries": int(totals[0]), "xg_entries": int(totals[1])})
        out.update(ex)
        out.update({"front_slot": int(scal[0]), "u_slot": int(scal[1]), "phase_b_level": int(scal[2]), "nranks": int(scal[4]), "rank": int(scal[5])})
        return out

    def __del__(self):
        if getattr(self, "handle", None):
            self._lib.lsa_nd_sym_destroy(self.handle)
            self.handle = None


def nd_order(A, leaf_size: int = 0, constraint=None) -> dict:
    an = NdAnalysis(A, leaf_size, constraint=constraint, order_only=True)
    ex = {"perm": np.empty(an.n, np.int32), "node_start": np.empty(an.ntree + 1, np.int32), "parent": np.empty(an.ntree, np.int32),
          "level": np.empty(an.ntree, np.int32)}
    an._lib.lsa_nd_sym_export(an.handle, _ptr(ex["perm"]), _ptr(ex["node_start"]), _ptr(ex["parent"]), _ptr(ex["level"]), None, None)
    return {"perm": ex["perm"].astype(np.int64), "first": ex["node_start"][:-1].copy(), "size": np.diff(ex["node_start"]).astype(np.int32),
            "parent": ex["parent"], "level": ex["level"]}


NDLU_BATCH_MAX = 16
NDLU_MULTI_MAX = 8
NDLU_MULTI_CHUNK = 256
_TRANS = {"N": 0, "T": 1, "H": 2}


class NdLu:

    def __init__(self, ctx: Context, C: CsrMatrix, leaf_size: int = 0, tree: dict | None = None):
        self.ctx, self._C = ctx, C
        h = ctypes.c_void_p()
        if tree is None:
            ctx.check(ctx._lib.lsa_ndlu_create(ctx.handle, C.handle, int(leaf_size), ctypes.byref(h)))
        else:
            first, size, parent = (np.ascontiguousarray(tree[k], dtype=np.int32) for k in ("first", "size", "parent"))
            owner = None if tree.get("owner") is None else np.ascontiguousarray(tree["owner"], dtype=np.int32)
            ctx.check(ctx._lib.lsa_ndlu_create_tree(ctx.handle, C.handle, len(parent), _ptr(first), _ptr(size), _ptr(parent),
                                                    None if owner is None else _ptr(owner), ctypes.byref(h)))
        self.handle = h
        self.n = C.shape[0]

    def refactor(self, C: CsrMatrix) -> None:
        self.ctx.check(self.ctx._lib.lsa_ndlu_refactor(self.ctx.handle, self.handle, C.handle))
        self._C = C

    def info(self) -> dict:
        nt, nl, mf, nla = _I32(0), _I32(0), _I32(0), _I32(0)
        fe, fre, ab = _I64(0), _I64(0), _I64(0)
        sa, sn = _DBL(0.0), _DBL(0.0)
        self.ctx._lib.lsa_ndlu_info(self.handle, ctypes.byref(nt), ctypes.byref(nl), ctypes.byref(mf), ctypes.byref(fe), ctypes.byref(fre),
                                    ctypes.byref(ab), ctypes.byref(nla), ctypes.byref(sa), ctypes.byref(sn))
        return {"tree_nodes": nt.value, "levels": nl.value, "max_front": mf.value, "factor_entries": fe.value, "front_entries": fre.value,
                "apply_bytes": ab.value, "apply_launches": nla.value, "seconds_analyse": sa.value, "seconds_numeric": sn.value}

    def sweep_levels(self) -> list[dict]:
        keys = ("nodes", "max_pivot", "fwd_rows", "bwd_rows", "fwd_tiles", "bwd_tiles")
        out = []
        for level in range(self.info()["levels"]):
            v = [_I32(0) for _ in keys]
            if self.ctx._lib.lsa_ndlu_sweep_level(self.handle, level, *[ctypes.byref(a) for a in v]) != 0:
                break
            out.append({k: a.value for k, a in zip(keys, v)})
        return out

    def solve(self, b: DeviceVector, x: DeviceVector) -> None:
        self.ctx.check(self.ctx._lib.lsa_ndlu_solve(self.ctx.handle, self.handle, b.handle, x.handle))

    @staticmethod
    def solve_batch(factors: "list[NdLu]", bs: "list[DeviceVector]", xs: "list[DeviceVector]") -> None:
        J = len(factors)
        if J == 0 or len(bs) != J or len(xs) != J:
            raise ValueError("solve_batch needs as many right-hand sides and outputs as factorisations (at least one)")
        if J > NDLU_BATCH_MAX:
            raise ValueError(f"solve_batch takes at most {NDLU_BATCH_MAX} factorisations, got {J}")
        ctx = factors[0].ctx
        if any(f.ctx is not ctx for f in factors) or any(v.ctx is not ctx for v in list(bs) + list(xs)):
            raise ValueError("solve_batch: the factorisations and vectors must live in one context")
        arr = lambda objs: (ctypes.c_void_p * J)(*[o.handle.value for o in objs])
        ctx.check(ctx._lib.lsa_ndlu_solve_batch(ctx.handle, J, arr(factors), arr(bs), arr(xs)))

    def solve_adjoint(self, b: DeviceVector, x: DeviceVector, conj: bool = True) -> None:
        self.ctx.check(self.ctx._lib.lsa_ndlu_solve_adjoint(self.ctx.handle, self.handle, int(conj), b.handle, x.handle))

    def time_solve(self, b: DeviceVector, x: DeviceVector, iters: int) -> float:
        ms = _DBL(0.0)
        self.ctx.check(self.ctx._lib.lsa_ndlu_solve_time(self.ctx.handle, self.handle, b.handle, x.handle, int(iters), ctypes.byref(ms)))
        return ms.value

    def _multi_args(self, B: DeviceVector, X: DeviceVector, nrhs: int, ldb, ldx, trans: str):
        if trans not in _TRANS:
            raise ValueError(f"trans must be 'N', 'T' or 'H', got {trans!r}")
        return (self.ctx.handle, self.handle, _TRANS[trans], int(nrhs), B.handle, int(self.n if ldb is None else ldb), X.handle,
                int(self.n if ldx is None else ldx))

    def solve_multi(self, B: DeviceVector, X: DeviceVector, nrhs: int, ldb: int | None = None, ldx: int | None = None, trans: str = "N") -> None:
        self.ctx.check(self.ctx._lib.lsa_ndlu_solve_multi(*self._multi_args(B, X, nrhs, ldb, ldx, trans)))

    def time_solve_multi(self, B: DeviceVector, X: DeviceVector, nrhs: int, iters: int, ldb: int | None = None, ldx: int | None = None,
                         trans: str = "N") -> float:
        ms = _DBL(0.0)
        self.ctx.check(self.ctx._lib.lsa_ndlu_solve_multi_time(*self._multi_args(B, X, nrhs, ldb, ldx, trans), int(iters), ctypes.byref(ms)))
        return ms.value

    def set_multi_transposed(self, on: bool) -> None:
        self.ctx.check(self.ctx._lib.lsa_ndlu_set_multi_transposed(self.ctx.handle, self.handle, int(bool(on))))

    def multi_info(self) -> dict:
        w, la, eb = _I32(0), _I32(0), _I64(0)
        self.ctx.check(self.ctx._lib.lsa_ndlu_multi_info(self.handle, ctypes.byref(w), ctypes.byref(eb), ctypes.byref(la)))
        return {"width": w.value, "extra_bytes": eb.value, "launches_per_pass": la.value}

    def inertia(self) -> tuple[int, int, int]:
        ng, ze, ps = _I64(0), _I64(0), _I64(0)
        self.ctx.check(self.ctx._lib.lsa_ndlu_inertia(self.ctx.handle, self.handle, ctypes.byref(ng), ctypes.byref(ze), ctypes.byref(ps)))
        return ng.value, ze.value, ps.value

    def __del__(self):
        if getattr(self, "handle", None) and getattr(self.ctx, "handle", None):
            self.ctx._lib.lsa_ndlu_destroy(self.handle)
            self.handle = None


def gmres(ctx: Context, C: CsrMatrix, pc: Ilu | None, b: DeviceVector, x: DeviceVector, *, rtol=1e-10, restart=200, maxit=2000,
          use_x0=False):
    its, rr = _I32(0), _DBL(0.0)
    rc = ctx._lib.lsa_gmres(ctx.handle, C.handle, pc.handle if pc else None, b.handle, x.handle, int(use_x0), float(rtol), int(restart),
                            int(maxit), ctypes.byref(its), ctypes.byref(rr))
    ctx.check(rc)
    return its.value, rr.value


class ShiftInvertOperator:

    def __init__(self, ctx: Context, A: CsrMatrix, M: CsrMatrix | None, sigma: complex, *, mode: int = 0, antishift: complex = 0.0,
                 ilu_levels: int = 0,
                 ilu_shift: float = 0.0, ksp_rtol: float = 1e-11, ksp_restart: int = 200, ksp_maxit: int = 2000, pc_type: int = 1,
# ... 654 lines not shown
```

Baseline: 599.6.

## Fuse GJ panel staging into finish launch and pair MFMA gemm kernels

In the numeric factorization, the stage kernel that copies pivot rows into the y-buffer is folded into the final Gauss-Jordan fused launch as extra blocks. The KIND 0 and KIND 2 MFMA gemm launches are merged into one paired kernel, and an optional 16-wide GJ panel path is added behind an environment variable. A launch counter is exposed through lsa_ndlu_info. The intent is to cut kernel launch count and per-launch overhead in refactorization, at the cost of a larger grid with mixed block roles and an API signature change.

```diff
diff --git a/include/lsa_hip.h b/include/lsa_hip.h
--- a/include/lsa_hip.h
+++ b/include/lsa_hip.h
@@ -117,7 +117,7 @@
 int lsa_ndlu_prepared_memory(lsa_ctx *ctx, int64_t *out);
 int lsa_ndlu_info(const lsa_ndlu *f, int32_t *ntree, int32_t *nlevels, int32_t *max_front, int64_t *factor_entries,
                   int64_t *front_entries, int64_t *apply_bytes, int32_t *apply_launches, double *seconds_analyse,
-                  double *seconds_numeric);
+                  double *seconds_numeric, int32_t *factor_launches);
 int lsa_ndlu_sweep_level(const lsa_ndlu *f, int32_t level, int32_t *nodes, int32_t *max_pivot, int32_t *fwd_rows, int32_t *bwd_rows,
                          int32_t *fwd_tiles, int32_t *bwd_tiles);
 
diff --git a/lsa-fw_amd/csrc/ndlu.hip b/lsa-fw_amd/csrc/ndlu.hip
--- a/lsa-fw_amd/csrc/ndlu.hip
+++ b/lsa-fw_amd/csrc/ndlu.hip
@@ -120,6 +120,9 @@
     f->ycap = kNB;
     const char* sbc = getenv("LSA_ND_SB_COLS");
     f->sb_cols = sbc && *sbc ? std::min(1024, std::max(kGT, atoi(sbc) / kGT * kGT)) : kSB;
+    const char* gp = getenv("LSA_ND_GJ_PANEL");
+    const int gpv = gp && *gp ? atoi(gp) : 0;
+    f->gj_panel = gpv == 8 || gpv == 16 ? gpv : 0;
 }
 
 bool nd_setup_ordered(const NdSymbolic& S) {
@@ -889,7 +892,7 @@
 }
 
 int lsa_ndlu_info(const lsa_ndlu* f, int32_t* ntree, int32_t* nlevels, int32_t* max_front, int64_t* factor_entries, int64_t* front_entries,
-                  int64_t* apply_bytes, int32_t* apply_launches, double* seconds_analyse, double* seconds_numeric) {
+                  int64_t* apply_bytes, int32_t* apply_launches, double* seconds_analyse, double* seconds_numeric, int32_t* factor_launches) {
     if (!f) return LSA_ERR_ARG;
     const NdSymbolic& S = f->S;
     if (ntree) *ntree = S.nt;
@@ -906,7 +909,8 @@
     if (apply_launches) *apply_launches = f->solve_launches;
     if (seconds_analyse) *seconds_analyse = f->seconds_analyse;
     if (seconds_numeric) *seconds_numeric = f->seconds_numeric;
-    return LSA_OK;
-}
-
-}
+    if (factor_launches) *factor_launches = f->factor_launches;
+    return LSA_OK;
+}
+
+}
diff --git a/lsa-fw_amd/csrc/ndlu_factor.hip b/lsa-fw_amd/csrc/ndlu_factor.hip
--- a/lsa-fw_amd/csrc/ndlu_factor.hip
+++ b/lsa-fw_amd/csrc/ndlu_factor.hip
@@ -1,4 +1,12 @@
 #include "ndlu_internal.h"
+
+#include <utility>
+
+#define ND_LAUNCH(f, ...)                   \
+    do {                                    \
+        ++(f)->factor_launches;             \
+        hipLaunchKernelGGL(__VA_ARGS__);    \
+    } while (0)
 
 namespace {
 
@@ -113,11 +121,42 @@
     return ((unsigned long long)__double_as_longlong(mag2) & ~0xFFFFull) | (unsigned long long)(65535 - row);
 }
 
+template <typename F, int... J>
+__device__ __forceinline__ void static_for_seq(F&& f, std::integer_sequence<int, J...>) {
+    (f(std::integral_constant<int, J>{}), ...);
+}
+template <int N, typename F>
+__device__ __forceinline__ void static_for(F&& f) {
+    static_for_seq(f, std::make_integer_sequence<int, N>{});
+}
+
+
+
+template <typename T>
+__device__ __forceinline__ void gj_stage_column(const NdNodeDev& nd, const T* front, const int32_t* ipiv, int32_t kb, int32_t kw, int32_t ycap,
+                                                int32_t c, int32_t c_hi, T* ybuf) {
+    const int32_t m = nd.m, ld = nd.f;
+    const int32_t nb = min(kw, m - kb);
+    if (nb <= 0 || m <= kNB || c >= min(m, c_hi)) return;
+    const T* a = front + nd.front_off;
+    T* yb = ybuf + (size_t)ycap * nd.piv_off;
+    const int32_t* pv = ipiv + nd.piv_off + kb;
+    int32_t j = 0;
+    for (; j + 4 <= nb; j += 4) {
+        const T v0 = a[(size_t)pv[j] * ld + c], v1 = a[(size_t)pv[j + 1] * ld + c], v2 = a[(size_t)pv[j + 2] * ld + c], v3 = a[(size_t)pv[j + 3] * ld + c];
+        yb[(size_t)j * m + c] = v0;
+        yb[(size_t)(j + 1) * m + c] = v1;
+        yb[(size_t)(j + 2) * m + c] = v2;
+        yb[(size_t)(j + 3) * m + c] = v3;
+    }
+    for (; j < nb; ++j) yb[(size_t)j * m + c] = a[(size_t)pv[j] * ld + c];
+}
 
 template <typename T, int NT, int RPT, int W>
 __global__ __launch_bounds__(NT) void nd_gj_fused_kernel(const int32_t* __restrict__ lvl_nodes, const NdNodeDev* __restrict__ nodes,
                                                          T* __restrict__ front, int32_t* __restrict__ ipiv, int32_t* __restrict__ rowq,
-                                                         int32_t kb, int32_t k0, int32_t kprev, int32_t* __restrict__ flag, double tiny2) {
+                                                         int32_t kb, int32_t k0, int32_t kprev, int32_t* __restrict__ flag, double tiny2,
+                                                         int32_t ystage, T* __restrict__ ybuf, int32_t c_hi) {
     __shared__ unsigned long long skey[W];
     __shared__ T prow_s[2][W];
     __shared__ int32_t prows[W];
@@ -128,6 +167,10 @@
     const int32_t m = nd.m, ld = nd.f;
     T* a = front + nd.front_off;
     const int tid = threadIdx.x, lane = tid & 63;
+    if (ystage > 0 && (int32_t)blockIdx.y >= ystage) {
+        gj_stage_column<T>(nd, front, ipiv, kb, kNB, kNB, ((int32_t)blockIdx.y - ystage) * NT + tid, c_hi, ybuf);
+        return;
+    }
     const int32_t wp = kprev >= 0 ? min(W, m - kprev) : 0;
     if (blockIdx.y > 0) {
         if (wp <= 0) return;
@@ -145,11 +188,11 @@
         T y[W];
 #pragma unroll
         for (int j = 0; j < W; ++j) y[j] = yprev[j][tid & 15];
-        constexpr int RL = NT / 16;
-        for (int32_t i0 = tid >> 4; i0 < m; i0 += 4 * RL) {
-            T cur[4], mult[4][W];
-#pragma unroll
-            for (int u = 0; u < 4; ++u) {
+        constexpr int RL = NT / 16, U = W > 8 ? 2 : 4;
+        for (int32_t i0 = tid >> 4; i0 < m; i0 += U * RL) {
+            T cur[U], mult[U][W];
+#pragma unroll
+            for (int u = 0; u < U; ++u) {
                 const int32_t i = i0 + u * RL;
                 const T* ai = a + (size_t)min(i, m - 1) * ld;
                 cur[u] = ai[c];
@@ -157,7 +200,7 @@
                 for (int j = 0; j < W; ++j) mult[u][j] = j < wp ? ai[kprev + j] : scalar_traits<T>::zero();
             }
 #pragma unroll
-            for (int u = 0; u < 4; ++u) {
+            for (int u = 0; u < U; ++u) {
                 const int32_t i = i0 + u * RL;
                 if (i >= m) break;
                 bool is_piv = false;
@@ -181,9 +224,11 @@
         pprev[tid] = tid < wp ? piv[kprev + tid] : -1;
     }
     __syncthreads();
-    if (wp > 0 && tid < W * W) {
-        const int j = tid / W, cc = tid % W;
-        yprev[j][cc] = (j < wp && cc < w) ? a[(size_t)pprev[j] * ld + k0 + cc] : scalar_traits<T>::zero();
+    if (wp > 0) {
+        for (int e = tid; e < W * W; e += NT) {
+            const int j = e / W, cc = e % W;
+            yprev[j][cc] = (j < wp && cc < w) ? a[(size_t)pprev[j] * ld + k0 + cc] : scalar_traits<T>::zero();
+        }
     }
     T r[RPT][W];
     bool used[RPT];
@@ -215,9 +260,9 @@
             }
         }
     }
-#pragma unroll
-    for (int jj = 0; jj < W; ++jj) {
-        if (jj >= w) break;
+    static_for<W>([&](auto jc) {
+        constexpr int jj = decltype(jc)::value;
+        if (jj >= w) return;
         unsigned long long key = 0ull;
 #pragma unroll
         for (int q = 0; q < RPT; ++q) {
@@ -270,7 +315,7 @@
 #pragma unroll
             for (int j = 0; j < W; ++j) fma_acc(r[q][j], nfm, prow[j]);
         }
-    }
+    });
 #pragma unroll
     for (int q = 0; q < RPT; ++q) {
         const int32_t i = tid + NT * q;
@@ -286,24 +331,8 @@
 __global__ __launch_bounds__(256) void nd_gj_stage_kernel(const int32_t* __restrict__ lvl_nodes, const NdNodeDev* __restrict__ nodes,
                                                           const T* __restrict__ front, const int32_t* __restrict__ ipiv, int32_t kb, int32_t kw,
                                                           int32_t ycap, int32_t c_lo, int32_t c_hi, T* __restrict__ ybuf) {
-    const int32_t t = lvl_nodes[blockIdx.x];
-    const NdNodeDev nd = nodes[t];
-    const int32_t m = nd.m, ld = nd.f;
-    const int32_t nb = min(kw, m - kb);
-    const int32_t c = c_lo + (int32_t)blockIdx.y * 256 + threadIdx.x;
-    if (nb <= 0 || m <= kNB || c >= min(m, c_hi)) return;
-    const T* a = front + nd.front_off;
-    T* yb = ybuf + (size_t)ycap * nd.piv_off;
-    const int32_t* pv = ipiv + nd.piv_off + kb;
-    int32_t j = 0;
-    for (; j + 4 <= nb; j += 4) {
-        const T v0 = a[(size_t)pv[j] * ld + c], v1 = a[(size_t)pv[j + 1] * ld + c], v2 = a[(size_t)pv[j + 2] * ld + c], v3 = a[(size_t)pv[j + 3] * ld + c];
-        yb[(size_t)j * m + c] = v0;
-        yb[(size_t)(j + 1) * m + c] = v1;
-        yb[(size_t)(j + 2) * m + c] = v2;
-        yb[(size_t)(j + 3) * m + c] = v3;
-    }
-    for (; j < nb; ++j) yb[(size_t)j * m + c] = a[(size_t)pv[j] * ld + c];
+    const NdNodeDev nd = nodes[lvl_nodes[blockIdx.x]];
+    gj_stage_column<T>(nd, front, ipiv, kb, kw, ycap, c_lo + (int32_t)blockIdx.y * 256 + (int32_t)threadIdx.x, c_hi, ybuf);
 }
 
 template <typename T>
@@ -663,11 +692,9 @@
 }
 
 template <typename T, int KIND>
-__global__ __launch_bounds__(256) void nd_gemm_mfma_kernel(const int32_t* __restrict__ tiles, const NdNodeDev* __restrict__ nodes,
-                                                           T* __restrict__ front, T* __restrict__ lfac, T* __restrict__ ufac) {
+__device__ __forceinline__ void gemm_mfma_tile(int32_t t, int32_t packed, const NdNodeDev* __restrict__ nodes, T* __restrict__ front,
+                                               T* __restrict__ lfac, T* __restrict__ ufac, MfmaTile<T>& sm) {
     constexpr int NPL = MfmaTile<T>::NPL;
-    __shared__ MfmaTile<T> sm;
-    const int32_t t = tiles[2 * blockIdx.x], packed = tiles[2 * blockIdx.x + 1];
     const int32_t tm = packed >> 16, tn = packed & 0xFFFF;
     const NdNodeDev nd = nodes[t];
     const int32_t m = nd.m, f = nd.f, b = f - m;
@@ -719,6 +746,23 @@
                 else *c = v;
             }
         }
+}
+
+template <typename T, int KIND>
+__global__ __launch_bounds__(256) void nd_gemm_mfma_kernel(const int32_t* __restrict__ tiles, const NdNodeDev* __restrict__ nodes,
+                                                           T* __restrict__ front, T* __restrict__ lfac, T* __restrict__ ufac) {
+    __shared__ MfmaTile<T> sm;
+    gemm_mfma_tile<T, KIND>(tiles[2 * blockIdx.x], tiles[2 * blockIdx.x + 1], nodes, front, lfac, ufac, sm);
+}
+
+template <typename T>
+__global__ __launch_bounds__(256) void nd_gemm_mfma_pair_kernel(const int32_t* __restrict__ tiles0, int32_t count0, const int32_t* __restrict__ tiles2,
+                                                                const NdNodeDev* __restrict__ nodes, T* __restrict__ front, T* __restrict__ lfac,
+                                                                T* __restrict__ ufac) {
+    __shared__ MfmaTile<T> sm;
+    const int32_t g = (int32_t)blockIdx.x;
+    if (g < count0) gemm_mfma_tile<T, 0>(tiles0[2 * g], tiles0[2 * g + 1], nodes, front, lfac, ufac, sm);
+    else gemm_mfma_tile<T, 2>(tiles2[2 * (g - count0)], tiles2[2 * (g - count0) + 1], nodes, front, lfac, ufac, sm);
 }
 
 template <typename T>
@@ -840,25 +884,32 @@
     };
     const int32_t kend = std::min(kb + kNB, L.max_m);
     const bool others = std::min(kNB, L.max_m - kb) > W;
+    constexpr bool between = 2 * W < kNB;
+    const bool outside = L.max_m > kNB;
     int32_t kprev = -1, active_prev = 0;
     for (int32_t k0 = kb; k0 < kend; k0 += W) {
         const int32_t active = active_at(k0);
         if (active == 0) break;
-        hipLaunchKernelGGL((nd_gj_fused_kernel<T, NT, RPT, W>), dim3(std::max(active, active_prev), others && kprev >= 0 ? 1 + kNB / 16 : 1), dim3(NT), 0, st, lv,
-                           f->d_nodes, front, f->d_ipiv, f->d_rowq, kb, k0, kprev, f->d_flag, tiny2);
+        ND_LAUNCH(f, (nd_gj_fused_kernel<T, NT, RPT, W>), dim3(std::max(active, active_prev), others && between && kprev >= 0 ? 1 + kNB / 16 : 1), dim3(NT), 0,
+                  st, lv, f->d_nodes, front, f->d_ipiv, f->d_rowq, kb, k0, kprev, f->d_flag, tiny2, 0, (T*)f->d_ybuf, 0);
         kprev = k0;
         active_prev = active;
     }
-    if (others && kprev >= 0)
-        hipLaunchKernelGGL((nd_gj_fused_kernel<T, NT, RPT, W>), dim3(active_prev, 1 + kNB / 16), dim3(NT), 0, st, lv, f->d_nodes, front, f->d_ipiv, f->d_rowq, kb,
-                           -1, kprev, f->d_flag, tiny2);
-    if (L.max_m > kNB) {
+    const bool finish = others && kprev >= 0;
+    const bool ride = finish && outside && f->gj_panel != 8;
+    if (finish) {
+        const int32_t ftiles = between ? kNB / 16 : (kprev - kb + 15) / 16;
+        ND_LAUNCH(f, (nd_gj_fused_kernel<T, NT, RPT, W>), dim3(ride ? active_at(kb) : active_prev, 1 + ftiles + (ride ? (L.max_m + NT - 1) / NT : 0)), dim3(NT),
+                  0, st, lv, f->d_nodes, front, f->d_ipiv, f->d_rowq, kb, -1, kprev, f->d_flag, tiny2, ride ? 1 + ftiles : 0, (T*)f->d_ybuf, L.max_m);
+    }
+    if (outside) {
         const int32_t active = active_at(kb);
-        hipLaunchKernelGGL((nd_gj_stage_kernel<T>), dim3(active, (L.max_m + 255) / 256), dim3(256), 0, st, lv, f->d_nodes, (const T*)front, f->d_ipiv, kb,
-                           kNB, kNB, 0, L.max_m, (T*)f->d_ybuf);
+        if (!ride)
+            ND_LAUNCH(f, (nd_gj_stage_kernel<T>), dim3(active, (L.max_m + 255) / 256), dim3(256), 0, st, lv, f->d_nodes, (const T*)front, f->d_ipiv, kb, kNB, kNB,
+                      0, L.max_m, (T*)f->d_ybuf);
         const int32_t tiles = (L.max_m + kGT - 1) / kGT;
-        hipLaunchKernelGGL((nd_gj_gemm_kernel<T>), dim3(active, tiles, tiles), dim3(256), 0, st, lv, f->d_nodes, front, f->d_rowq, kb, (const T*)f->d_ybuf, 0, 0,
-                           0, 0, 0);
+        ND_LAUNCH(f, (nd_gj_gemm_kernel<T>), dim3(active, tiles, tiles), dim3(256), 0, st, lv, f->d_nodes, front, f->d_rowq, kb, (const T*)f->d_ybuf, 0, 0,
+                  0, 0, 0);
     }
 }
 
@@ -869,18 +920,18 @@
     const int32_t active = (int32_t)(std::lower_bound(L.sorted_m.begin(), L.sorted_m.end(), kb, std::greater<int32_t>()) - L.sorted_m.begin());
     if (active == 0) return;
     int32_t sets = (L.max_m + tp_first<T>::rows - 1) / tp_first<T>::rows;
-    hipLaunchKernelGGL((nd_tp_round_kernel<T, true, false>), dim3(active, sets), dim3(256), 0, st, lv, f->d_nodes, front, f->d_ipiv, f->d_rowq, kb, 0,
-                       (const int32_t*)nullptr, f->d_cand[0], (T*)nullptr, f->d_flag, tiny2);
+    ND_LAUNCH(f, (nd_tp_round_kernel<T, true, false>), dim3(active, sets), dim3(256), 0, st, lv, f->d_nodes, front, f->d_ipiv, f->d_rowq, kb, 0,
+              (const int32_t*)nullptr, f->d_cand[0], (T*)nullptr, f->d_flag, tiny2);
     int src = 0;
     for (int32_t round = 0;; ++round) {
         const int32_t groups = (sets + kTA - 1) / kTA;
         if (groups == 1) {
-            hipLaunchKernelGGL((nd_tp_round_kernel<T, false, true>), dim3(active, 1), dim3(256), 0, st, lv, f->d_nodes, front, f->d_ipiv, f->d_rowq, kb, round,
-                               (const int32_t*)f->d_cand[src], (int32_t*)nullptr, (T*)f->d_dinv, f->d_flag, tiny2);
+            ND_LAUNCH(f, (nd_tp_round_kernel<T, false, true>), dim3(active, 1), dim3(256), 0, st, lv, f->d_nodes, front, f->d_ipiv, f->d_rowq, kb, round,
+                      (const int32_t*)f->d_cand[src], (int32_t*)nullptr, (T*)f->d_dinv, f->d_flag, tiny2);
             break;
         }
-        hipLaunchKernelGGL((nd_tp_round_kernel<T, false, false>), dim3(active, groups), dim3(256), 0, st, lv, f->d_nodes, front, f->d_ipiv, f->d_rowq, kb, round,
-                           (const int32_t*)f->d_cand[src], f->d_cand[src ^ 1], (T*)nullptr, f->d_flag, tiny2);
+        ND_LAUNCH(f, (nd_tp_round_kernel<T, false, false>), dim3(active, groups), dim3(256), 0, st, lv, f->d_nodes, front, f->d_ipiv, f->d_rowq, kb, round,
+                  (const int32_t*)f->d_cand[src], f->d_cand[src ^ 1], (T*)nullptr, f->d_flag, tiny2);
         src ^= 1;
         sets = groups;
     }
@@ -900,12 +951,12 @@
     const int32_t sbw = wide ? f->sb_cols : kNB, ycap = f->ycap;
     const int32_t tiles = (L.max_m + kGT - 1) / kGT;
     auto stage = [&](int32_t active, int32_t k0, int32_t kw, int32_t c_lo, int32_t c_hi) {
-        hipLaunchKernelGGL((nd_gj_stage_kernel<T>), dim3(active, (c_hi - c_lo + 255) / 256), dim3(256), 0, st, lv, f->d_nodes, (const T*)front, f->d_ipiv, k0, kw,
-                           ycap, c_lo, c_hi, (T*)f->d_ybuf);
+        ND_LAUNCH(f, (nd_gj_stage_kernel<T>), dim3(active, (c_hi - c_lo + 255) / 256), dim3(256), 0, st, lv, f->d_nodes, (const T*)front, f->d_ipiv, k0, kw,
+                  ycap, c_lo, c_hi, (T*)f->d_ybuf);
     };
     auto update = [&](int32_t active, int32_t k0, int32_t kw, int32_t zt0, int32_t ztn, int32_t only_lo, int32_t only_hi, int32_t skip_lo, int32_t skip_hi) {
-        hipLaunchKernelGGL((nd_gj_update_kernel<T>), dim3(active, tiles, ztn), dim3(256), 0, st, lv, f->d_nodes, front, f->d_rowq, k0, kw, (const T*)f->d_ybuf,
-                           ycap, only_lo, only_hi, skip_lo, skip_hi, zt0);
+        ND_LAUNCH(f, (nd_gj_update_kernel<T>), dim3(active, tiles, ztn), dim3(256), 0, st, lv, f->d_nodes, front, f->d_rowq, k0, kw, (const T*)f->d_ybuf,
+                  ycap, only_lo, only_hi, skip_lo, skip_hi, zt0);
     };
     launch_tournament<T>(f, L, 0, tiny2, st);
     for (int32_t sb0 = 0; sb0 < L.max_m; sb0 += sbw) {
@@ -914,8 +965,8 @@
         for (int32_t kb = sb0; kb < sb1; kb += kNB) {
             const int32_t active = active_at(kb);
             if (active == 0) break;
-            hipLaunchKernelGGL((nd_tp_colblock_kernel<T>), dim3(active, (L.max_m + 255) / 256), dim3(256), 0, st, lv, f->d_nodes, front, f->d_rowq, kb,
-                               (const T*)f->d_dinv);
+            ND_LAUNCH(f, (nd_tp_colblock_kernel<T>), dim3(active, (L.max_m + 255) / 256), dim3(256), 0, st, lv, f->d_nodes, front, f->d_rowq, kb,
+                      (const T*)f->d_dinv);
             if (sb1 - sb0 > kNB) {
                 stage(active, kb, kNB, sb0, sb1);
                 update(active, kb, kNB, sb0 / kGT, (sb1 + kGT - 1) / kGT - sb0 / kGT, sb0, sb1, 0, 0);
@@ -953,6 +1004,7 @@
     T* upd = (T*)f->d_upd;
     int rc0 = LSA_OK;
     double max2 = 0.0;
+    f->factor_launches = 0;
     {
         auto head = [&]() -> int {
             LSA_HIP_CHECK(ctx, hipMemsetAsync(f->d_rowq, 0xFF, (size_t)std::max<int32_t>(S.n, 1) * sizeof(int32_t), st));
@@ -960,7 +1012,7 @@
             LSA_HIP_CHECK(ctx, hipMemsetAsync(f->d_maxabs, 0, sizeof(unsigned long long), st));
             if (S.nnz > 0) {
                 const int blocks = (int)std::min<int64_t>((S.nnz + 255) / 256, (int64_t)ctx->num_cu * 2);
-                hipLaunchKernelGGL((nd_maxabs2_kernel<T>), dim3(blocks), dim3(256), 0, st, S.nnz, (const T*)C->val, f->d_maxabs);
+                ND_LAUNCH(f, (nd_maxabs2_kernel<T>), dim3(blocks), dim3(256), 0, st, S.nnz, (const T*)C->val, f->d_maxabs);
             }
             unsigned long long mbits = 0;
             LSA_HIP_CHECK(ctx, hipMemcpyAsync(&mbits, f->d_maxabs, sizeof mbits, hipMemcpyDeviceToHost, st));
@@ -984,12 +1036,12 @@
         LSA_HIP_CHECK(ctx, hipMemsetAsync(f->d_work, 0, (size_t)L.work_entries * sizeof(T), st));
         if (L.asm_count > 0) {
             const int blocks = (int)std::min<int64_t>((L.asm_count + 255) / 256, (int64_t)ctx->num_cu * 16);
-            hipLaunchKernelGGL((nd_assemble_kernel<T>), dim3(blocks), dim3(256), 0, st, L.asm_count, (const T*)C->val, f->d_asm_src + L.asm_begin,
-                               f->d_asm_dst + L.asm_begin, front);
+            ND_LAUNCH(f, (nd_assemble_kernel<T>), dim3(blocks), dim3(256), 0, st, L.asm_count, (const T*)C->val, f->d_asm_src + L.asm_begin,
+                      f->d_asm_dst + L.asm_begin, front);
         }
         for (const TileList& e : L.ext)
             if (e.count > 0)
-                hipLaunchKernelGGL((nd_extend_add_kernel<T>), dim3(e.count), dim3(256), 0, st, tl + 2 * e.off, f->d_nodes, f->d_cmap, front, (const T*)upd);
+                ND_LAUNCH(f, (nd_extend_add_kernel<T>), dim3(e.count), dim3(256), 0, st, tl + 2 * e.off, f->d_nodes, f->d_cmap, front, (const T*)upd);
         for (const auto& step : L.xsteps) {
             T* stage = (T*)f->d_xstage;
             int64_t stride = 0;
@@ -1009,13 +1061,18 @@
             for (int r = 0; r < S.nranks; ++r) {
                 const NdChunk::XPiece& pc = step[(size_t)r];
                 if (pc.nrows <= 0) continue;
-                hipLaunchKernelGGL((nd_extend_add_staged_kernel<T>), dim3((pc.nrows + 15) / 16), dim3(256), 0, st, f->d_nodes, f->d_cmap, front,
-                                   (const T*)(stage + (size_t)r * (size_t)stride), pc.child, pc.row0, pc.nrows);
+                ND_LAUNCH(f, (nd_extend_add_staged_kernel<T>), dim3((pc.nrows + 15) / 16), dim3(256), 0, st, f->d_nodes, f->d_cmap, front,
+                          (const T*)(stage + (size_t)r * (size_t)stride), pc.child, pc.row0, pc.nrows);
             }
         }
         if (L.max_m >= f->tp_min) LSA_CHECK(launch_level_tp<T>(ctx, f, L, tiny2));
         for (int32_t kb = 0; kb < L.max_m && L.max_m < f->tp_min; kb += kNB) {
-            if (L.max_m <= 64) launch_block<T, 64, 1, 8>(ctx, f, L, kb, tiny2);
+            if (f->gj_panel == 16 && L.max_m <= 512) {
+                if (L.max_m <= 64) launch_block<T, 64, 1, 16>(ctx, f, L, kb, tiny2);
+                else if (L.max_m <= 128) launch_block<T, 128, 1, 16>(ctx, f, L, kb, tiny2);
+                else if (L.max_m <= 256) launch_block<T, 256, 1, 16>(ctx, f, L, kb, tiny2);
+                else launch_block<T, 512, 1, 16>(ctx, f, L, kb, tiny2);
+            } else if (L.max_m <= 64) launch_block<T, 64, 1, 8>(ctx, f, L, kb, tiny2);
             else if (L.max_m <= 128) launch_block<T, 128, 1, 8>(ctx, f, L, kb, tiny2);
             else if (L.max_m <= 256) launch_block<T, 256, 1, 8>(ctx, f, L, kb, tiny2);
             else if (L.max_m <= 512) launch_block<T, 512, 1, 8>(ctx, f, L, kb, tiny2);
@@ -1026,24 +1083,30 @@
             else launch_block<T, 1024, 16, 1>(ctx, f, L, kb, tiny2);
         }
         if (L.unperm.count > 0)
-            hipLaunchKernelGGL((nd_unperm_kernel<T>), dim3(L.unperm.count), dim3(256), 0, st, tl + 2 * L.unperm.off, f->d_nodes, front, f->d_ipiv,
-                               f->d_rowq, lfac);
+            ND_LAUNCH(f, (nd_unperm_kernel<T>), dim3(L.unperm.count), dim3(256), 0, st, tl + 2 * L.unperm.off, f->d_nodes, front, f->d_ipiv,
+                      f->d_rowq, lfac);
         auto product = [&](auto kind) {
             constexpr int KIND = decltype(kind)::value;
             if (L.gemm[KIND].count == 0) return;
-            hipLaunchKernelGGL((nd_gemm_mfma_kernel<T, KIND>), dim3(L.gemm[KIND].count), dim3(256), 0, st, tl + 2 * L.gemm[KIND].off, f->d_nodes, front, lfac, ufac);
+            ND_LAUNCH(f, (nd_gemm_mfma_kernel<T, KIND>), dim3(L.gemm[KIND].count), dim3(256), 0, st, tl + 2 * L.gemm[KIND].off, f->d_nodes, front, lfac, ufac);
         };
-        product(std::integral_constant<int, 0>{});
-        product(std::integral_constant<int, 1>{});
-        product(std::integral_constant<int, 2>{});
+        if (f->gj_panel != 8 && L.gemm[0].count > 0 && L.gemm[2].count > 0) {
+            ND_LAUNCH(f, (nd_gemm_mfma_pair_kernel<T>), dim3(L.gemm[0].count + L.gemm[2].count), dim3(256), 0, st, tl + 2 * L.gemm[0].off, (int32_t)L.gemm[0].count,
+                      tl + 2 * L.gemm[2].off, f->d_nodes, front, lfac, ufac);
+            product(std::integral_constant<int, 1>{});
+        } else {
+            product(std::integral_constant<int, 0>{});
+            product(std::integral_constant<int, 1>{});
+            product(std::integral_constant<int, 2>{});
+        }
         if (L.save.count > 0)
-            hipLaunchKernelGGL((nd_save_update_kernel<T>), dim3(L.save.count), dim3(256), 0, st, tl + 2 * L.save.off, f->d_nodes, (const T*)front, upd);
+            ND_LAUNCH(f, (nd_save_update_kernel<T>), dim3(L.save.count), dim3(256), 0, st, tl + 2 * L.save.off, f->d_nodes, (const T*)front, upd);
     }
     if (f->top.s > 0)
         for (int q = 0, t0 = 0; q < 2; t0 += f->top_tiles[q++])
             if (f->top_tiles[q] > 0)
-                hipLaunchKernelGGL((nd_top_gemm_kernel<T>), dim3(f->top_tiles[q]), dim3(256), 0, st, f->d_top_tiles + 2 * t0, f->d_top_jobs, f->d_cmap,
-                                   (const T*)lfac, (const T*)ufac, (T*)f->d_top, f->top.s);
+                ND_LAUNCH(f, (nd_top_gemm_kernel<T>), dim3(f->top_tiles[q]), dim3(256), 0, st, f->d_top_tiles + 2 * t0, f->d_top_jobs, f->d_cmap,
+                          (const T*)lfac, (const T*)ufac, (T*)f->d_top, f->top.s);
     if (!exchanged && S.nranks > 1 && f->xupd_slot > 0)
         LSA_CHECK(k_allgather_inplace(ctx, f->d_upd, (size_t)f->xupd_slot * sizeof(T)));
     int32_t hflag[4] = {0, 0, 0, 0};
@@ -1082,7 +1145,7 @@
         const double eps = atof(pe);
         if (eps != 0.0 && f->ufac_entries > 0) {
             const int blocks = (int)std::min<int64_t>((f->ufac_entries + 255) / 256, (int64_t)ctx->num_cu * 16);
-            hipLaunchKernelGGL((nd_scale_kernel<T>), dim3(blocks), dim3(256), 0, st, f->ufac_entries, ufac, 1.0 + eps);
+            ND_LAUNCH(f, (nd_scale_kernel<T>), dim3(blocks), dim3(256), 0, st, f->ufac_entries, ufac, 1.0 + eps);
             LSA_HIP_CHECK(ctx, hipStreamSynchronize(st));
         }
     }
diff --git a/lsa-fw_amd/csrc/ndlu_internal.h b/lsa-fw_amd/csrc/ndlu_internal.h
--- a/lsa-fw_amd/csrc/ndlu_internal.h
+++ b/lsa-fw_amd/csrc/ndlu_internal.h
@@ -146,6 +146,8 @@
     int32_t sb_min = 1 << 30;
     int32_t sb_cols = 128;
     int32_t ycap = 32;
+    int32_t gj_panel = 0;
+    int32_t factor_launches = 0;
     hipStream_t side = nullptr;
     hipEvent_t ev_panel = nullptr, ev_pivots = nullptr;
     double seconds_analyse = 0.0, seconds_numeric = 0.0;
diff --git a/lsa-fw_amd/csrc/solver.hip b/lsa-fw_amd/csrc/solver.hip
--- a/lsa-fw_amd/csrc/solver.hip
+++ b/lsa-fw_amd/csrc/solver.hip
@@ -647,7 +647,7 @@
             rc = lsa_ndlu_create(ctx, fac_src, 0, &op->nd);
         if (rc == LSA_OK && op->nd) {
             double sa = 1.0;
-            (void)lsa_ndlu_info(op->nd, nullptr, nullptr, nullptr, nullptr, nullptr, nullptr, nullptr, &sa, nullptr);
+            (void)lsa_ndlu_info(op->nd, nullptr, nullptr, nullptr, nullptr, nullptr, nullptr, nullptr, &sa, nullptr, nullptr);
             op->st.analysis_reused = sa == 0.0 ? 1 : 0;
         }
         if (rc == LSA_ERR_OOM) {
@@ -1446,7 +1446,7 @@
         if (lead < 0) break;
         int rc = lsa_ensure_scratch(ctx, 0, cells * (colb + 2 * sizeof(double)));
         int32_t sweep_launches = 0;
-        (void)lsa_ndlu_info(ks[lead]->op->nd, nullptr, nullptr, nullptr, nullptr, nullptr, nullptr, &sweep_launches, nullptr, nullptr);
+        (void)lsa_ndlu_info(ks[lead]->op->nd, nullptr, nullptr, nullptr, nullptr, nullptr, nullptr, &sweep_launches, nullptr, nullptr, nullptr);
         for (int32_t s = 0; s < rounds && rc == LSA_OK; ++s) {
             int32_t R = 0, jr[kKrylovGroupMax], fr[kKrylovGroupMax];
             lsa_ndlu* nd[kKrylovGroupMax];
diff --git a/lsa-fw_amd/lsa_hip/__init__.py b/lsa-fw_amd/lsa_hip/__init__.py
--- a/lsa-fw_amd/lsa_hip/__init__.py
+++ b/lsa-fw_amd/lsa_hip/__init__.py
@@ -208,7 +208,8 @@
     "lsa_ndlu_set_multi_transposed": (ctypes.c_int, [_P, _P, ctypes.c_int]),
     "lsa_ndlu_multi_info": (ctypes.c_int, [_P, ctypes.POINTER(_I32), ctypes.POINTER(_I64), ctypes.POINTER(_I32)]),
     "lsa_ndlu_info": (ctypes.c_int, [_P, ctypes.POINTER(_I32), ctypes.POINTER(_I32), ctypes.POINTER(_I32), ctypes.POINTER(_I64),
-                                     ctypes.POINTER(_I64), ctypes.POINTER(_I64), ctypes.POINTER(_I32), ctypes.POINTER(_DBL), ctypes.POINTER(_DBL)]),
+                                     ctypes.POINTER(_I64), ctypes.POINTER(_I64), ctypes.POINTER(_I32), ctypes.POINTER(_DBL), ctypes.POINTER(_DBL),
+                                     ctypes.POINTER(_I32)]),
     "lsa_ndlu_sweep_level": (ctypes.c_int, [_P, _I32] + [ctypes.POINTER(_I32)] * 6),
     "lsa_gmres": (ctypes.c_int, [_P, _P, _P, _P, _P, ctypes.c_int, _DBL, ctypes.c_int, ctypes.c_int, ctypes.POINTER(_I32), ctypes.POINTER(_DBL)]),
     "lsa_op_create": (ctypes.c_int, [_P, _P, _P, _DBL * 2, ctypes.c_int, ctypes.POINTER(lsa_op_options), _PP]),
@@ -754,13 +755,14 @@
         self._C = C
 
     def info(self) -> dict:
-        nt, nl, mf, nla = _I32(0), _I32(0), _I32(0), _I32(0)
+        nt, nl, mf, nla, nfl = _I32(0), _I32(0), _I32(0), _I32(0), _I32(0)
         fe, fre, ab = _I64(0), _I64(0), _I64(0)
         sa, sn = _DBL(0.0), _DBL(0.0)
         self.ctx._lib.lsa_ndlu_info(self.handle, ctypes.byref(nt), ctypes.byref(nl), ctypes.byref(mf), ctypes.byref(fe), ctypes.byref(fre),
-                                    ctypes.byref(ab), ctypes.byref(nla), ctypes.byref(sa), ctypes.byref(sn))
+                                    ctypes.byref(ab), ctypes.byref(nla), ctypes.byref(sa), ctypes.byref(sn), ctypes.byref(nfl))
         return {"tree_nodes": nt.value, "levels": nl.value, "max_front": mf.value, "factor_entries": fe.value, "front_entries": fre.value,
-                "apply_bytes": ab.value, "apply_launches": nla.value, "seconds_analyse": sa.value, "seconds_numeric": sn.value}
+                "apply_bytes": ab.value, "apply_launches": nla.value, "seconds_analyse": sa.value, "seconds_numeric": sn.value,
+                "factor_launches": nfl.value}
 
     def sweep_levels(self) -> list[dict]:
         keys = ("nodes", "max_pivot", "fwd_rows", "bwd_rows", "fwd_tiles", "bwd_tiles")
```

After: 612.4 (median of 6 runs). +2.1%, better.
